# abb128/april-asr

Hardware: AMD Instinct MI355X
Metric: audio_seconds_per_second (concurrent 16 kHz sessions x 1/RTF), aprilv0_en-us-sized streaming RNN-T (higher is better)
Workload: dtype f32

## Files before the change

### april_asr_amd/csrc/engine.cc

```cpp
#include "engine.h"
#include <array>
#include <algorithm>
#include <cmath>
#include <chrono>
#include <cstdlib>
#include <cstring>
#include "common.h"
#include "env.h"

namespace aprilx {

static size_t align64(size_t x) { return (x + 63) & ~(size_t)63; }

void plan_layout(const NetDims &d, bool has_dec_conv_b, PackedLayout &L)
{
    L.dims = d;
    L.has_dec_conv_b = has_dec_conv_b;
    L.vocab_pad = (d.vocab + 31) & ~31;
    size_t off = 0;
    auto take = [&](size_t n) { size_t o = off; off = align64(off + n); return o; };
    L.k3 = (d.conv_ch[1] * 9 + 63) & ~63;
    L.conv_w[0] = take((size_t)d.conv_ch[0] * 9); L.conv_b[0] = take((size_t)d.conv_ch[0]);
    L.conv_w[1] = take((size_t)d.conv_ch[1] * d.conv_ch[0] * 9); L.conv_b[1] = take((size_t)d.conv_ch[1]);
    L.conv_w[2] = take((size_t)L.k3 * d.conv_ch[2]); L.conv_b[2] = take((size_t)d.conv_ch[2]);
    L.w_embed = take((size_t)d.embed_in * d.d_model); L.b_embed = take((size_t)d.d_model);
    L.layers.resize((size_t)d.n_layers);
    for (auto &l : L.layers) {
        l.wg = take((size_t)2 * d.d_model * 4 * d.hidden); l.bg = take((size_t)4 * d.hidden);
        l.whr = take((size_t)d.hidden * d.d_model);
        l.wff1 = take((size_t)d.d_model * d.ffn); l.bff1 = take((size_t)d.ffn);
        l.wff2 = take((size_t)d.ffn * d.d_model); l.bff2 = take((size_t)d.d_model);
    }
    L.w_encproj = take((size_t)d.d_model * d.joiner); L.b_encproj = take((size_t)d.joiner);
    L.emb = take((size_t)d.vocab * d.d_model);
    L.dec_conv = take((size_t)d.d_model * (d.d_model / d.dec_groups) * d.context);
    L.dec_conv_b = take((size_t)d.d_model);
    L.w_decproj = take((size_t)d.d_model * d.joiner); L.b_decproj = take((size_t)d.joiner);
    L.w_out = take((size_t)d.joiner * L.vocab_pad); L.b_out = take((size_t)L.vocab_pad);
    L.total = off;
}

std::vector<std::pair<size_t, size_t>> gemm_sections(const PackedLayout &L)
{
    const NetDims &d = L.dims;
    std::vector<std::pair<size_t, size_t>> v;
    v.emplace_back(L.w_embed, (size_t)d.embed_in * d.d_model);
    for (const PackedLayout::Layer &o : L.layers) {
        v.emplace_back(o.wg, (size_t)2 * d.d_model * 4 * d.hidden); v.emplace_back(o.whr, (size_t)d.hidden * d.d_model);
        v.emplace_back(o.wff1, (size_t)d.d_model * d.ffn); v.emplace_back(o.wff2, (size_t)d.ffn * d.d_model);
    }
    v.emplace_back(L.w_encproj, (size_t)d.d_model * d.joiner); v.emplace_back(L.w_decproj, (size_t)d.d_model * d.joiner);
    v.emplace_back(L.w_out, (size_t)d.joiner * L.vocab_pad);
    return v;
}

static void pack_mfma(const float *W, int K, int N, int Npad, const std::vector<int> *colmap, float *dst)
{
    const int KB = K / 16, NTt = Npad / 16;
    for (int t = 0; t < NTt; ++t)
        for (int kb = 0; kb < KB; ++kb)
            for (int lane = 0; lane < 64; ++lane) {
                const int np = t * 16 + (lane & 15);
                const int src = np < N ? (colmap ? (*colmap)[(size_t)np] : np) : -1;
                float *o = dst + (((size_t)t * KB + kb) * 64 + lane) * 4;
                for (int j = 0; j < 4; ++j) {
                    const int k = kb * 16 + (lane >> 4) * 4 + j;
                    o[j] = src >= 0 ? W[(size_t)k * N + src] : 0.0f;
                }
            }
}

void pack_weights(const HostModel &m, PackedLayout &L, std::vector<float> &blob)
{
    const NetDims &d = L.dims;
    blob.assign(L.total, 0.0f);
    float *B = blob.data();
    for (int i = 0; i < 3; ++i) {
        if (i < 2) memcpy(B + L.conv_w[i], m.conv_w[i].data(), m.conv_w[i].size() * 4);
        memcpy(B + L.conv_b[i], m.conv_b[i].data(), m.conv_b[i].size() * 4);
    }
    {
        const int kreal = d.conv_ch[1] * 9, c2 = d.conv_ch[2];
        std::vector<float> w3((size_t)L.k3 * c2, 0.0f);
        for (int o = 0; o < c2; ++o) for (int k = 0; k < kreal; ++k) w3[(size_t)k * c2 + o] = m.conv_w[2][(size_t)o * kreal + k];
        pack_mfma(w3.data(), L.k3, c2, c2, nullptr, B + L.conv_w[2]);
    }
    {
        const int c2 = d.conv_ch[2], F = d.f_out;
        std::vector<float> we((size_t)d.embed_in * d.d_model);
        for (int c = 0; c < c2; ++c) for (int f = 0; f < F; ++f)
            memcpy(&we[((size_t)f * c2 + c) * d.d_model], &m.w_embed[((size_t)c * F + f) * d.d_model], (size_t)d.d_model * 4);
        pack_mfma(we.data(), d.embed_in, d.d_model, d.d_model, nullptr, B + L.w_embed);
    }
    memcpy(B + L.b_embed, m.b_embed.data(), (size_t)d.d_model * 4);
    L.embed_eps = m.embed_norm_eps;
    L.norm_eps.resize((size_t)d.n_layers);
    std::vector<int> gmap((size_t)4 * d.hidden);
    for (int u = 0; u < d.hidden; ++u) for (int g = 0; g < 4; ++g) gmap[(size_t)u * 4 + g] = g * d.hidden + u;
    for (int l = 0; l < d.n_layers; ++l) {
        const LayerWeights &lw = m.layers[(size_t)l];
        const PackedLayout::Layer &o = L.layers[(size_t)l];
        pack_mfma(lw.w_gates.data(), 2 * d.d_model, 4 * d.hidden, 4 * d.hidden, &gmap, B + o.wg);
        for (int n = 0; n < 4 * d.hidden; ++n) B[o.bg + n] = lw.b_gates[(size_t)gmap[(size_t)n]];
        pack_mfma(lw.w_hr.data(), d.hidden, d.d_model, d.d_model, nullptr, B + o.whr);
        pack_mfma(lw.w_ff1.data(), d.d_model, d.ffn, d.ffn, nullptr, B + o.wff1);
        memcpy(B + o.bff1, lw.b_ff1.data(), (size_t)d.ffn * 4);
        pack_mfma(lw.w_ff2.data(), d.ffn, d.d_model, d.d_model, nullptr, B + o.wff2);
        memcpy(B + o.bff2, lw.b_ff2.data(), (size_t)d.d_model * 4);
        L.norm_eps[(size_t)l] = lw.norm_eps;
    }
    pack_mfma(m.w_encproj.data(), d.d_model, d.joiner, d.joiner, nullptr, B + L.w_encproj);
    memcpy(B + L.b_encproj, m.b_encproj.data(), (size_t)d.joiner * 4);
    memcpy(B + L.emb, m.emb.data(), m.emb.size() * 4);
    memcpy(B + L.dec_conv, m.dec_conv.data(), m.dec_conv.size() * 4);
    if (!m.dec_conv_b.empty()) memcpy(B + L.dec_conv_b, m.dec_conv_b.data(), m.dec_conv_b.size() * 4);
    pack_mfma(m.w_decproj.data(), d.d_model, d.joiner, d.joiner, nullptr, B + L.w_decproj);
    memcpy(B + L.b_decproj, m.b_decproj.data(), (size_t)d.joiner * 4);
    pack_mfma(m.w_out.data(), d.joiner, d.vocab, L.vocab_pad, nullptr, B + L.w_out);
    memcpy(B + L.b_out, m.b_out.data(), (size_t)d.vocab * 4);
}

template <typename T> static T *dmalloc(size_t n) { HipLegacyLock legacy; T *p = nullptr; HIP_CHECK(hipMalloc((void **)&p, std::max<size_t>(n, 1) * sizeof(T))); return p; }
template <typename T> static T *hmalloc(size_t n) { HipLegacyLock legacy; T *p = nullptr; HIP_CHECK(hipHostMalloc((void **)&p, std::max<size_t>(n, 1) * sizeof(T), hipHostMallocDefault)); return p; }

std::recursive_mutex &hip_legacy_mutex() { static std::recursive_mutex m; return m; }

static int pick_kz(int K, int N, int kblk = 16)
{
    int kz = 256 / std::max(1, N / 16);
    kz = std::max(1, std::min(kz, 8));
    while (kz > 1 && ((K / kblk) / kz < 4 || (K / kblk) % (4 * kz) != 0)) kz >>= 1;
    return kz;
}

Engine::Engine(const EngineConfig &cfg, const PackedLayout &layout, const float *blob_host, const float *blob_device,
               const ModelParams &params, const FbankHostTables &ft, const std::vector<uint8_t> &tok_class)
    : cfg_(cfg), L_(layout), P_(params)
{
    HipLegacyLock legacy;
    HIP_CHECK(hipSetDevice(cfg_.device));
    HIP_CHECK(hipStreamCreateWithFlags(&stream_, hipStreamNonBlocking));
    HIP_CHECK(hipStreamCreateWithFlags(&f_stream_, hipStreamNonBlocking));
    HIP_CHECK(hipStreamCreateWithFlags(&s_stream_, hipStreamNonBlocking));
    search_stream_ = stream_;
    for (int i = 0; i < 32; ++i) { hipEvent_t e; HIP_CHECK(hipEventCreateWithFlags(&e, hipEventDisableTiming)); join_ev_.push_back(e); }
    split_streams_ = std::max(0, std::min(2, env_int("APRIL_SPLIT_STREAMS", 2)));
    const NetDims &d = L_.dims;
    w_ = dmalloc<float>(L_.total);
    if (blob_device) HIP_CHECK(hipMemcpy(w_, blob_device, L_.total * 4, hipMemcpyDeviceToDevice));
    else if (blob_host) HIP_CHECK(hipMemcpy(w_, blob_host, L_.total * 4, hipMemcpyHostToDevice));

    const size_t S = (size_t)cfg_.max_slots, MB = (size_t)cfg_.max_batch;
    ring_frames_ = std::max(P_.segment_size * 32, env_int("APRIL_RING_FRAMES", 8192));
    h_ = dmalloc<float>((size_t)d.n_layers * S * d.d_model);
    c_ = dmalloc<float>((size_t)d.n_layers * S * d.hidden);
    if (!env_str("APRIL_RING_FRAMES")) {
        size_t free_b = 0, total_b = 0;
        if (hipMemGetInfo(&free_b, &total_b) == hipSuccess && free_b > 0) {
            const size_t per_frame = S * (size_t)d.mel * sizeof(float);
            const size_t fit = (free_b / 4) / per_frame;
            if (fit < (size_t)ring_frames_) {
                const int shrunk = std::max(P_.segment_size * 32, (int)std::min<size_t>(fit, 8192) / 64 * 64);
                LOGW("engine: %zu MB of feature rings (%d frames x %zu slots) exceed a quarter of the %zu MB free on device %d: %d frames per session",
                     per_frame * (size_t)ring_frames_ >> 20, ring_frames_, S, free_b >> 20, cfg_.device, shrunk);
                ring_frames_ = shrunk;
            }
        } else (void)hipGetLastError();
        float *p = nullptr;
        if (hipMalloc((void **)&p, S * ring_frames_ * d.mel * sizeof(float)) == hipSuccess) ring_ = p;
        else {
            (void)hipGetLastError();
            const size_t asked = S * (size_t)ring_frames_ * d.mel * sizeof(float);
            ring_frames_ = std::max(P_.segment_size * 32, 2048);
            LOGW("engine: no room for %zu MB of feature rings, falling back to %d frames per session", asked >> 20, ring_frames_);
        }
    }
    if (!ring_) ring_ = dmalloc<float>(S * ring_frames_ * d.mel);
    eout_ = dmalloc<float>(S * d.joiner);
    dout_ = dmalloc<float>(S * d.joiner);
    gstate_ = dmalloc<GreedyState>(S);
    HIP_CHECK(hipMemset(h_, 0, (size_t)d.n_layers * S * d.d_model * 4));
    HIP_CHECK(hipMemset(c_, 0, (size_t)d.n_layers * S * d.hidden * 4));
    HIP_CHECK(hipMemset(ring_, 0, S * ring_frames_ * d.mel * 4));
    HIP_CHECK(hipMemset(eout_, 0, S * d.joiner * 4));
    HIP_CHECK(hipMemset(dout_, 0, S * d.joiner * 4));
    {
        std::vector<GreedyState> init(S);
        for (auto &g : init) { g.ctx0 = P_.blank_id; g.ctx1 = P_.blank_id; g.last_tok = -1; g.last_emit_ms = 0; }
        HIP_CHECK(hipMemcpy(gstate_, init.data(), S * sizeof(GreedyState), hipMemcpyHostToDevice));
    }
    cls_ = dmalloc<uint8_t>((size_t)d.vocab);
    HIP_CHECK(hipMemcpy(cls_, tok_class.data(), (size_t)d.vocab, hipMemcpyHostToDevice));

    kz_embed_ = pick_kz(d.embed_in, d.d_model);
    kz_hr_ = pick_kz(d.hidden, d.d_model);
    kz_ff2_ = pick_kz(d.ffn, d.d_model);
    kz_proj_ = pick_kz(d.d_model, d.joiner);
    kz_out_ = pick_kz(d.joiner, L_.vocab_pad);
    {
        const bool want = cfg_.precision == 1 && env_int("APRIL_F16_TILE", 1) != 0;
        f16_tile_ = want && d.d_model % 128 == 0 && d.hidden % 128 == 0 && d.ffn % 128 == 0 && d.hidden % 16 == 0;
        if (f16_tile_) {
            kzx_hr_ = pick_kz(d.hidden, d.d_model, 32); kzx_ff2_ = pick_kz(d.ffn, d.d_model, 32);
            for (int p = 0; p < 2; ++p) y16_buf_[p] = dmalloc<uint16_t>(MB * d.d_model);
            y16_ = y16_buf_[0];
            for (int p = 0; p < 2; ++p) { xb16_buf_[p] = dmalloc<uint16_t>(MB * d.d_model); u16_buf_[p] = dmalloc<uint16_t>(MB * d.hidden); ff16_buf_[p] = dmalloc<uint16_t>(MB * d.ffn); }
            xb16_ = xb16_buf_[0]; u16_ = u16_buf_[0]; ff16_ = ff16_buf_[0];
            h16_ = dmalloc<uint16_t>((size_t)d.n_layers * S * d.d_model);
            HIP_CHECK(hipMemset(h16_, 0, (size_t)d.n_layers * S * d.d_model * 2));
        }
    }
    ws_mstride_ = cfg_.max_batch;
    const size_t ws_n = (size_t)std::max({kz_embed_ * d.d_model, kz_hr_ * d.d_model, kz_ff2_ * d.d_model, kz_proj_ * d.joiner, kz_out_ * L_.vocab_pad});
    ws_ = dmalloc<float>(ws_n * MB);
    ws_g_ = dmalloc<float>((size_t)std::max(kz_proj_ * d.joiner, kz_out_ * L_.vocab_pad) * MB);
    xin_ = dmalloc<float>(MB * d.embed_in);
    a3_ = dmalloc<float>(MB * d.f_out * L_.k3);
    HIP_CHECK(hipMemset(a3_, 0, MB * d.f_out * L_.k3 * 4));
    for (int p = 0; p < 2; ++p) { y_buf_[p] = dmalloc<float>(MB * d.d_model); ssq_buf_[p] = dmalloc<float>(MB * (d.d_model / SSQ_COLS)); }
    y_ = y_buf_[0]; ssq_ = ssq_buf_[0];
    ws_fe_ = dmalloc<float>((size_t)kz_embed_ * d.d_model * MB);
    ws_sr_ = dmalloc<float>((size_t)std::max(kz_proj_ * d.joiner, d.d_model) * MB);
    for (int p = 0; p < 2; ++p) { xb_buf_[p] = dmalloc<float>(MB * d.d_model); u_buf_[p] = dmalloc<float>(MB * d.hidden); ff_buf_[p] = dmalloc<float>(MB * d.ffn); }
    xb_ = xb_buf_[0]; u_ = u_buf_[0]; ff_ = ff_buf_[0];
    ramp_mode_ = env_int("APRIL_RAMP_MERGE", 1);
    if (ramp_mode_ < 0 || ramp_mode_ > 2) ramp_mode_ = 1;
    ramp_d_ = dmalloc<RampState>(1); HIP_CHECK(hipMemset(ramp_d_, 0, sizeof(RampState)));
    de_ = dmalloc<float>(MB * d.d_model);
    HIP_CHECK(hipMemset(de_, 0, MB * d.d_model * 4));
    logits_ = dmalloc<float>(3 * MB * d.vocab);
    logits_h_ = hmalloc<float>(3 * MB * d.vocab);
    ring_cap_ = std::max<size_t>((size_t)1 << 20, 3 * MB * 8 + 2 * S); ring_h_ = hmalloc<int>(2 * ring_cap_);
    step_cap_ = 1 << 14; step_off_h_ = hmalloc<int>((size_t)2 * step_cap_); rec_off_h_ = hmalloc<int>((size_t)2 * step_cap_);
    rec_cap_ = std::max<size_t>((size_t)1 << 20, 3 * MB * 8); rec_d_ = dmalloc<StepRecord>(2 * rec_cap_); rec_h_ = hmalloc<StepRecord>(2 * rec_cap_);
    for (int i = 0; i < 2; ++i) HIP_CHECK(hipEventCreateWithFlags(&flight_done_[i], hipEventDisableTiming));
    counter_d_ = dmalloc<int>(1);
    for (int p = 0; p < 2; ++p) {
        rec_off_buf_[p] = dmalloc<int>(1); flags_buf_[p] = dmalloc<int>(8); step_buf_[p] = dmalloc<int>(4 * MB);
        HIP_CHECK(hipMemset(rec_off_buf_[p], 0, 4)); HIP_CHECK(hipMemset(flags_buf_[p], 0, 32));
    }
    rec_off_d_ = rec_off_buf_[0]; flags_d_ = flags_buf_[0]; step_d_ = step_buf_[0];
    active_d_ = dmalloc<int>(MB); dirty_d_ = dmalloc<int>(MB);
    dec_slots_d_ = dmalloc<int>(std::max(S, MB));
    HIP_CHECK(hipMemset(counter_d_, 0, 4));

    upload_tables(ft);
    use_graphs_ = env_int("APRIL_NO_GRAPHS", 0) == 0;
    if (const int n = env_int("APRIL_GRAPH_CACHE_CAP", 0))
        step_graphs_.cap = lm_graphs_.cap = lm_search_graphs_.cap = sw_plan_cap_ = (size_t)std::max(n, 2), sw_graphs_.cap = 4 * sw_plan_cap_;
    free_.reserve(S);
    for (int i = cfg_.max_slots - 1; i >= 0; --i) free_.push_back(i);
    LOGI("engine: device %d, %d slots, max batch %d, weights %.1f MB, kz(embed,hr,ff2,proj,out)=%d,%d,%d,%d,%d",
         cfg_.device, cfg_.max_slots, cfg_.max_batch, L_.total * 4.0 / 1e6, kz_embed_, kz_hr_, kz_ff2_, kz_proj_, kz_out_);
}

void Engine::finish_weights()
{
    HipLegacyLock legacy;
    HIP_CHECK(hipSetDevice(cfg_.device));
    if (cfg_.precision == 1 && !wh_) {
        wh_ = dmalloc<uint16_t>(L_.total);
        for (const auto &sec : gemm_sections(L_)) launch_cvt_f16(w_ + sec.first, wh_ + sec.first, sec.second, nullptr);
        if (f16_tile_) {
            const NetDims &d = L_.dims;
            wx_ = dmalloc<uint16_t>(L_.total);
            for (const PackedLayout::Layer &o : L_.layers) {
                launch_repack_x32(w_ + o.wg, wx_ + o.wg, 2 * d.d_model, 4 * d.hidden, nullptr);
                launch_repack_x32(w_ + o.whr, wx_ + o.whr, d.hidden, d.d_model, nullptr);
                launch_repack_x32(w_ + o.wff1, wx_ + o.wff1, d.d_model, d.ffn, nullptr);
                launch_repack_x32(w_ + o.wff2, wx_ + o.wff2, d.ffn, d.d_model, nullptr);
            }
        }
        HIP_CHECK(hipDeviceSynchronize());
    }
    if (!conv_wt_) {
        const NetDims &d = L_.dims;
        conv_wt_ = dmalloc<float>((size_t)9 * d.conv_ch[0] + (size_t)9 * d.conv_ch[0] * d.conv_ch[1]);
        launch_conv_weight_transpose(w_ + L_.conv_w[0], w_ + L_.conv_w[1], d.conv_ch[0], d.conv_ch[1], conv_wt_, conv_wt_ + (size_t)9 * d.conv_ch[0], nullptr);
        HIP_CHECK(hipDeviceSynchronize());
    }
    build_dec_table();
}

void Engine::build_dec_table()
{
    if (dec_table_) return;
    const NetDims &d = L_.dims;
    const size_t limit_mb = (size_t)std::max(0, env_int("APRIL_DEC_TABLE_MB", 2048));
    const size_t rows = (size_t)d.vocab * (size_t)d.vocab;
    if (d.context != 2 || rows * (size_t)d.joiner * 4 > limit_mb * 1024 * 1024 || rows * (size_t)d.joiner * 4 >= ((size_t)1 << 32)) return;
    const int MB = cfg_.max_batch;
    float *table = dmalloc<float>(rows * (size_t)d.joiner);
    std::vector<int> iota((size_t)MB), ctx((size_t)MB * 2);
    for (int i = 0; i < MB; ++i) iota[(size_t)i] = i;
    int *ctx_d = dmalloc<int>((size_t)MB * 2);
    HIP_CHECK(hipMemcpy(dec_slots_d_, iota.data(), (size_t)MB * 4, hipMemcpyHostToDevice));
    for (size_t base = 0; base < rows; base += (size_t)MB) {
        const int n = (int)std::min<size_t>((size_t)MB, rows - base);
        for (int i = 0; i < n; ++i) { const size_t r = base + (size_t)i; ctx[(size_t)2 * i] = (int)(r / (size_t)d.vocab); ctx[(size_t)2 * i + 1] = (int)(r % (size_t)d.vocab); }
        HIP_CHECK(hipMemcpy(ctx_d, ctx.data(), (size_t)n * 8, hipMemcpyHostToDevice));
        DecEmbedArgs a; a.dec = dec_params(); a.ctx = ctx_d; a.M = n; a.out = de_; a.ldo = d.d_model;
        launch_dec_embed(a, stream_);
        run_decproj(n, dec_slots_d_, nullptr, nullptr, 1, table + base * (size_t)d.joiner);
        HIP_CHECK(hipStreamSynchronize(stream_));
    }
    (void)hipFree(ctx_d);
    dec_table_ = table;
    LOGI("engine: decoder table %zu rows x %d (%.0f MB)", rows, d.joiner, rows * (double)d.joiner * 4 / 1e6);
}

Engine::~Engine()
{
    HipLegacyLock legacy;
    (void)hipSetDevice(cfg_.device);
    (void)hipStreamSynchronize(f_stream_); (void)hipStreamSynchronize(stream_); (void)hipStreamSynchronize(s_stream_);
    dump_stream_trace();
    if (ramp_d_ && ramp_eligible_.load() > 0) {
        unsigned h = 0;
        if (hipMemcpy(&h, &ramp_d_->hosted, sizeof h, hipMemcpyDeviceToHost) == hipSuccess) LOGI("engine: ramp merge: %u of %llu hostable split feeds were hosted by their predecessor", h, (unsigned long long)ramp_eligible_.load());
    }
    for (StreamTrace &t : trace_) for (hipEvent_t e : t.ev) if (e) (void)hipEventDestroy(e);
    if (trace_base_) (void)hipEventDestroy(trace_base_);
    for (hipEvent_t e : join_ev_) (void)hipEventDestroy(e);
    for (auto &e : ev_pool_) { (void)hipEventDestroy(e.a); (void)hipEventDestroy(e.b); }
    drop_graphs(); free_sw_plans(); if (gclk_slots_) (void)hipFree(gclk_slots_);
    if (lm_stream_) { (void)hipStreamSynchronize(lm_stream_); (void)hipStreamDestroy(lm_stream_); }
    for (hipEvent_t e : lm_events_) (void)hipEventDestroy(e);
    if (zargs_h_) { (void)hipHostFree(zargs_h_); (void)hipFree(zargs_d_); }
    for (int i = 0; i < 3; ++i) if (zargs_done_[i]) (void)hipEventDestroy(zargs_done_[i]);
    for (void *p : {(void *)lm_now_d_, (void *)lm_rows_d_, (void *)lm_rec_off_d_}) if (p) (void)hipFree(p);
    if (conf_k_d_) (void)hipFree(conf_k_d_);
    if (conf_d_) (void)hipFree(conf_d_);
    if (conf_k_h_) (void)hipHostFree(conf_k_h_);
    if (conf_h_) (void)hipHostFree(conf_h_);
    for (auto &b : bias_sets_) if (b.dev) (void)hipFree(b.dev);
    for (void *p : {(void *)bias_set_d_, (void *)bias_state_d_, (void *)bias_desc_d_}) if (p) (void)hipFree(p);
    for (void *p : {(void *)bias_set_h_, (void *)bias_desc_h_}) if (p) (void)hipHostFree(p);
    if (opt_d_) (void)hipFree(opt_d_);
    if (opt_h_) (void)hipHostFree(opt_h_);
    if (ws_g_) (void)hipFree(ws_g_);
    if (conv_wt_) (void)hipFree(conv_wt_);
    if (dec_table_) (void)hipFree(dec_table_);
    if (p_lm_) (void)hipFree(p_lm_);
    for (int p = 0; p < 2; ++p)
        for (void *q : {(void *)eout_lm_buf_[p], (void *)y16_buf_[p], (void *)y_buf_[p], (void *)ssq_buf_[p], (void *)xb_buf_[p], (void *)u_buf_[p], (void *)ff_buf_[p],
                        (void *)xb16_buf_[p], (void *)u16_buf_[p], (void *)ff16_buf_[p], (void *)rec_off_buf_[p], (void *)flags_buf_[p], (void *)step_buf_[p]}) if (q) (void)hipFree(q);
    if (ws_fe_) (void)hipFree(ws_fe_);
    if (ws_sr_) (void)hipFree(ws_sr_);
    for (void *p : {(void *)wx_, (void *)h16_, (void *)ramp_d_}) if (p) (void)hipFree(p);
    for (void *p : {(void *)w_, (void *)wh_, (void *)h_, (void *)c_, (void *)ring_, (void *)eout_, (void *)dout_, (void *)gstate_, (void *)cls_, (void *)ws_, (void *)xin_,
                    (void *)a3_, (void *)de_, (void *)logits_, (void *)rec_d_, (void *)counter_d_,
                    (void *)active_d_, (void *)dirty_d_, (void *)dec_slots_d_,
                    (void *)ds_desc_[0], (void *)ds_desc_[1], (void *)ds_pcm_[0], (void *)ds_pcm_[1]})
        if (p) (void)hipFree(p);
    for (void *p : {(void *)ring_h_, (void *)step_off_h_, (void *)rec_off_h_, (void *)rec_h_, (void *)logits_h_, (void *)hs_desc_[0], (void *)hs_desc_[1], (void *)hs_pcm_[0], (void *)hs_pcm_[1]})
        if (p) (void)hipHostFree(p);
    for (int b = 0; b < 2; ++b) if (fb_done_[b]) (void)hipEventDestroy(fb_done_[b]);
    for (int b = 0; b < 2; ++b) if (flight_done_[b]) (void)hipEventDestroy(flight_done_[b]);
    for (void *p : table_allocs_) (void)hipFree(p);
    (void)hipStreamDestroy(stream_); (void)hipStreamDestroy(f_stream_); (void)hipStreamDestroy(s_stream_);
}

void Engine::upload_tables(const FbankHostTables &ft)
{
    auto up = [&](const void *src, size_t bytes) {
        void *p = nullptr;
        HIP_CHECK(hipMalloc(&p, std::max<size_t>(bytes, 16)));
        if (bytes) HIP_CHECK(hipMemcpy(p, src, bytes, hipMemcpyHostToDevice));
        table_allocs_.push_back(p);
        return p;
    };
    ft_.window = (const float *)up(ft.window.data(), ft.window.size() * 4);
    ft_.mel = (const float *)up(ft.mel.data(), ft.mel.size() * 4);
    ft_.mel_lo = (const int *)up(ft.mel_lo.data(), ft.mel_lo.size() * 4);
    ft_.mel_hi = (const int *)up(ft.mel_hi.data(), ft.mel_hi.size() * 4);
    ft_.nfct = (int)ft.factors.size();
    for (int k = 0; k < ft_.nfct; ++k) {
        ft_.fct[k] = ft.factors[(size_t)k];
        ft_.tw[k] = (const double *)up(ft.tw[(size_t)k].data(), ft.tw[(size_t)k].size() * 8);
        ft_.tws[k] = ft.tws[(size_t)k].empty() ? nullptr : (const double *)up(ft.tws[(size_t)k].data(), ft.tws[(size_t)k].size() * 8);
    }
    ft_.padded = ft.padded; ft_.nbins = ft.nbins;
    pad_value_ = ft.pad_value;
}

int Engine::alloc_slot()
{
    std::lock_guard<std::mutex> g(slot_mu_);
    if (free_.empty() && !zero_pending_.empty()) zero_pending_slots();
    if (free_.empty()) return -1;
    const int s = free_.back();
    free_.pop_back();
    ++live_;
    return s;
}

void Engine::zero_pending_slots()
{
    if (zero_pending_.empty()) return;
    if (hipSetDevice(cfg_.device) == hipSuccess) {
        std::lock_guard<std::mutex> cg(capture_mu_);
        m_touched();
        const NetDims &d = L_.dims;
        for (size_t o = 0; o < zero_pending_.size(); o += 64) {
            ZeroSlotArgs z;
            z.h = h_; z.c = c_; z.n_layers = d.n_layers; z.slots = (size_t)cfg_.max_slots; z.d_model = d.d_model; z.hidden = d.hidden;
            z.eout = eout_; z.dout = dout_; z.joiner = d.joiner; z.state = gstate_; z.blank = P_.blank_id; z.h16 = h16_;
            z.n_list = (int)std::min<size_t>(64, zero_pending_.size() - o);
            for (int i = 0; i < z.n_list; ++i) z.list[i] = zero_pending_[o + (size_t)i];
            launch_zero_slot(z, stream_);
        }
    }
    for (int s : zero_pending_) free_.push_back(s);
    zero_pending_.clear();
}

void Engine::free_slot(int slot)
{
    if (conf_ever_.load(std::memory_order_relaxed)) set_slot_confidence(slot, 0);
    if (bias_ever_.load(std::memory_order_relaxed)) set_slot_bias(slot, nullptr);
    if (opt_ever_.load(std::memory_order_relaxed)) set_slot_search_options(slot, SearchOpt{0u, 0.0f});
    std::lock_guard<std::mutex> g(slot_mu_);
    zero_pending_.push_back(slot);
    --live_;
    if (zero_pending_.size() >= 256) zero_pending_slots();
}

void Engine::sync_streams()
{
    HIP_CHECK(hipStreamSynchronize(f_stream_)); HIP_CHECK(hipStreamSynchronize(stream_)); HIP_CHECK(hipStreamSynchronize(s_stream_));
}

void Engine::sync()
{
    m_touched();
    sync_streams();
    f_unseen_by_m_ = s_unseen_by_m_ = m_unseen_by_f_ = m_unseen_by_s_ = false;
    if (profiling_) collect_timing();
}

template <typename Chain> static hipGraphExec_t capture_graph(hipStream_t st, Chain &&chain)
{
    hipGraph_t graph = nullptr;
    hipGraphExec_t exec = nullptr;
    HipLegacyLock capture_guard;
    HIP_CHECK(hipStreamBeginCapture(st, hipStreamCaptureModeRelaxed));
    chain();
    HIP_CHECK(hipStreamEndCapture(st, &graph));
    HIP_CHECK(hipGraphInstantiate(&exec, graph, nullptr, nullptr, 0));
    HIP_CHECK(hipGraphDestroy(graph));
    return exec;
}

void GraphCache::clear()
{
    if (!map_.empty()) LOGI("engine: %s graphs emptied (%zu entries)", name, map_.size());
    for (auto &g : map_) (void)hipGraphExecDestroy(g.second);
    map_.clear(); uses_.clear();
}

template <typename Chain> hipGraphExec_t Engine::cached_graph(GraphCache &cache, const GraphCache::Key &key, hipStream_t st, Chain &&chain)
{
    if (!cache.find(key)) cache.insert(key, capture_graph(st, chain));
    return cache.find(key);
}

template <typename Capture> void Engine::capture_both_parities(Capture &&capture)
{
    const int par = flight_parity_;
    m_touched();
    for (int q : {1 - par, par}) { select_parity(q); capture(); }
}

Engine::StreamTrace *Engine::trace_slot()
{
    static const char *path = env_str("APRIL_STREAM_TRACE");
    if (!path) return nullptr;
    if (!trace_base_) { HIP_CHECK(hipEventCreate(&trace_base_)); HIP_CHECK(hipEventRecord(trace_base_, stream_)); }
    if (trace_.size() >= 4096) return nullptr;
    trace_.emplace_back();
    StreamTrace &t = trace_.back();
    for (hipEvent_t &e : t.ev) HIP_CHECK(hipEventCreate(&e));
    return &t;
}

void Engine::dump_stream_trace()
{
    const char *path = env_str("APRIL_STREAM_TRACE");
    if (!path || trace_.empty()) return;
    FILE *f = fopen(path, "w");
    if (!f) return;
    fprintf(f, "# one line per split feed; times in us since the first split feed; FE = index fetch + conv + embed on stream F, LY = layer wavefront on M, SR = encoder_proj + search on S\n");
    fprintf(f, "# feed sessions chunks  FE_start FE_end  LY_start LY_end  SR_start SR_end   overlap: FE inside the previous feed's LY window? SR inside the next feed's LY window?\n");
    std::vector<std::array<float, 6>> ts;
    for (StreamTrace &t : trace_) {
        std::array<float, 6> a{};
        bool ok = t.used;
        for (int i = 0; i < 6 && ok; ++i) ok = hipEventElapsedTime(&a[(size_t)i], trace_base_, t.ev[i]) == hipSuccess;
        if (ok) ts.push_back(a); else (void)hipGetLastError();
    }
    for (size_t i = 0; i < ts.size(); ++i) {
        const auto &a = ts[i];
        const bool fe_in_prev = i > 0 && a[0] * 1e3f < ts[i - 1][3] * 1e3f && a[1] * 1e3f > ts[i - 1][2] * 1e3f;
        const bool sr_in_next = i + 1 < ts.size() && a[5] > ts[i + 1][2] && a[4] < ts[i + 1][3];
        fprintf(f, "%4zu %5d %2d  %10.1f %10.1f  %10.1f %10.1f  %10.1f %10.1f   %s %s\n", i, trace_[i].m, trace_[i].T, a[0] * 1e3, a[1] * 1e3, a[2] * 1e3, a[3] * 1e3, a[4] * 1e3, a[5] * 1e3,
                fe_in_prev ? "FE<prevLY" : "-", sr_in_next ? "SR<nextLY" : "-");
    }
    fclose(f);
}

void Engine::join(hipStream_t waiter, hipStream_t src)
{
    hipEvent_t e = join_ev_[join_pos_++ % join_ev_.size()];
    HIP_CHECK(hipEventRecord(e, src));
    HIP_CHECK(hipStreamWaitEvent(waiter, e, 0));
}

void Engine::general_prologue()
{
    m_touched();
    if (f_unseen_by_m_) { join(stream_, f_stream_); f_unseen_by_m_ = false; }
    if (s_unseen_by_m_) { join(stream_, s_stream_); s_unseen_by_m_ = false; }
    m_unseen_by_f_ = m_unseen_by_s_ = true;
    flight_tail_s_ = false;
}

void Engine::set_profiling(bool on) { std::lock_guard<std::mutex> cg(capture_mu_); sync(); profiling_ = on; }
void Engine::reset_timing() { for (auto &t : timing_) t = KernelTiming(); }
void Engine::set_gates_clock(bool on)
{
    std::lock_guard<std::mutex> cg(capture_mu_);
    HIP_CHECK(hipSetDevice(cfg_.device));
    sync();
    if (on) {
        if (!gclk_slots_) gclk_slots_ = dmalloc<unsigned long long>((size_t)GCLK_SLOTS * STAMP_WORDS);
        HIP_CHECK(hipMemsetAsync(gclk_slots_, 0, (size_t)GCLK_SLOTS * STAMP_WORDS * 8, stream_));
        HIP_CHECK(hipStreamSynchronize(stream_));
        gclk_ms_ = 0; gclk_launches_ = 0; gclk_rows_ = 0;
        for (int i = 0; i < 4; ++i) { gclk_ms_n_[i] = 0; gclk_launches_n_[i] = 0; }
        gclk_ = true;
        return;
    }
    collect_gates_clock(); gclk_ = false;
}
void Engine::collect_gates_clock()
{
    if (!gclk_ || !gclk_slots_) return;
    std::vector<unsigned long long> h((size_t)GCLK_SLOTS * STAMP_WORDS);
    HIP_CHECK(hipMemcpyAsync(h.data(), gclk_slots_, h.size() * 8, hipMemcpyDeviceToHost, stream_)); HIP_CHECK(hipStreamSynchronize(stream_));
    for (auto &kv : sw_plans_)
        for (size_t i = 0; i < kv.second.stamp_slots.size(); ++i) {
            const auto &sl = kv.second.stamp_slots[i];
            const unsigned long long ticks = h[(size_t)sl.first * STAMP_WORDS + 2], n = h[(size_t)sl.first * STAMP_WORDS + 3];
            gclk_ms_ += (double)ticks * 1e-5; gclk_launches_ += (long)n; gclk_rows_ += (long)n * sl.second;
            const int bn = std::min(std::max(kv.second.stamp_n[i], 1), 4) - 1;
            gclk_ms_n_[bn] += (double)ticks * 1e-5; gclk_launches_n_[bn] += (long)n;
        }
}
void Engine::timed_begin(int cls)
{
    ++launch_count_;
    if (!profiling_) return;
    if (ev_used_ == ev_pool_.size()) { Ev e; HIP_CHECK(hipEventCreate(&e.a)); HIP_CHECK(hipEventCreate(&e.b)); e.cls = cls; ev_pool_.push_back(e); }
    ev_pool_[ev_used_].cls = cls;
    if (cls == T_GATES) gemm_profile_next_launch(ev_pool_[ev_used_].a, ev_pool_[ev_used_].b);
    else HIP_CHECK(hipEventRecord(ev_pool_[ev_used_].a, stream_));
}
void Engine::timed_end(int cls)
{
    if (!profiling_) return;
    if (cls == T_GATES) {
        if (gemm_profile_pending()) { gemm_profile_next_launch(nullptr, nullptr); return; }
    } else HIP_CHECK(hipEventRecord(ev_pool_[ev_used_].b, stream_));
    ++ev_used_;
}
void Engine::collect_timing()
{
    for (size_t i = 0; i < ev_used_; ++i) {
        float ms = 0;
        if (hipEventElapsedTime(&ms, ev_pool_[i].a, ev_pool_[i].b) == hipSuccess) { timing_[ev_pool_[i].cls].ms += ms; timing_[ev_pool_[i].cls].launches++; }
    }
    ev_used_ = 0;
}

void Engine::fbank(int n_frames, const FbankFrameDesc *desc, const std::pair<const int16_t *, size_t> *parts, size_t n_parts, size_t n_pcm, HostPool *pool)
{
    const int n_rs = n_frames > 0 ? std::max(rs_n_, 0) : 0;
    ResampleDesc *rs = rs_desc_;
    const std::pair<const int16_t *, size_t> *in_parts = rs_in_parts_;
    const size_t n_in_parts = n_rs ? rs_n_in_parts_ : 0, n_in = n_rs ? rs_n_in_ : 0;
    rs_n_ = 0;
    const int n_dc = n_frames > 0 ? std::max(dc_n_, 0) : 0;
    const DecodeDesc *dc = dc_desc_;
    const std::pair<const uint8_t *, size_t> *raw_parts = dc_raw_parts_;
    const size_t n_raw_parts = n_dc ? dc_n_raw_parts_ : 0, n_raw = n_dc ? dc_n_raw_ : 0;
    const size_t raw_units = n_dc ? (n_raw + 1) / 2 + 8 : 0;
    dc_n_ = 0;
    if (n_frames <= 0) return;
    HIP_CHECK(hipSetDevice(cfg_.device));
    for (int i = 0; i < n_rs; ++i) rs[i].taps = resample_table(rs_specs_[i]);
    if (n_frames > desc_cap_ || n_pcm + n_in + raw_units > pcm_cap_ || (size_t)n_rs > rs_cap_ || (size_t)n_dc > dc_cap_) {
        sync();
        HipLegacyLock regrow_guard;
        for (int b = 0; b < 2; ++b) {
            if (hs_desc_[b]) { (void)hipHostFree(hs_desc_[b]); (void)hipFree(ds_desc_[b]); }
            if (hs_pcm_[b]) { (void)hipHostFree(hs_pcm_[b]); (void)hipFree(ds_pcm_[b]); }
        }
        desc_cap_ = std::max({n_frames * 2, desc_cap_, 1024});
        pcm_cap_ = std::max({(n_pcm + n_in + raw_units) * 2, pcm_cap_, (size_t)1 << 16});
        rs_cap_ = std::max({(size_t)n_rs * 2, rs_cap_, n_rs ? (size_t)256 : (size_t)0});
        dc_cap_ = std::max({(size_t)n_dc * 2, dc_cap_, n_dc ? (size_t)256 : (size_t)0});
        const size_t units = pcm_cap_ + 8 + ((size_t)desc_cap_ * sizeof(FbankFrameDesc) + 1) / 2 + 8 + rs_cap_ * sizeof(ResampleDesc) / 2
                             + 8 + dc_cap_ * sizeof(DecodeDesc) / 2;
        for (int b = 0; b < 2; ++b) {
            hs_pcm_[b] = hmalloc<int16_t>(units); ds_pcm_[b] = dmalloc<int16_t>(units);
            hs_desc_[b] = nullptr; ds_desc_[b] = nullptr;
            if (!fb_done_[b]) HIP_CHECK(hipEventCreateWithFlags(&fb_done_[b], hipEventDisableTiming));
        }
    }
    const int b = fb_flip_;
    fb_flip_ ^= 1;
    HIP_CHECK(hipEventSynchronize(fb_done_[b]));
    const size_t woff = ((n_pcm + n_in) * sizeof(int16_t) + 15) / 16 * 16;
    const size_t doff = (woff + n_raw + 15) / 16 * 16;
    const size_t roff = (doff + (size_t)n_frames * sizeof(FbankFrameDesc) + 15) / 16 * 16;
    const size_t coff = (roff + (size_t)n_rs * sizeof(ResampleDesc) + 15) / 16 * 16;
    const size_t bytes = n_dc ? coff + (size_t)n_dc * sizeof(DecodeDesc)
                              : (n_rs ? roff + (size_t)n_rs * sizeof(ResampleDesc) : doff + (size_t)n_frames * sizeof(FbankFrameDesc));
    char *hs = reinterpret_cast<char *>(hs_pcm_[b]);
    memcpy(hs + doff, desc, (size_t)n_frames * sizeof(FbankFrameDesc));
    ResampleArgs ra;
    if (n_rs) {
        ResampleDesc *hr = reinterpret_cast<ResampleDesc *>(hs + roff);
        int64_t blocks = 0, lds = 0;
        for (int i = 0; i < n_rs; ++i) {
            hr[i] = rs[i];
            hr[i].in_off += (int32_t)n_pcm;
            blocks = std::max<int64_t>(blocks, (rs[i].out_cnt + kResampleBlock - 1) / kResampleBlock);
            lds = std::max<int64_t>(lds, resample_lds_floats(rs[i].L, rs[i].M, rs[i].K));
        }
        ra.n_desc = n_rs; ra.max_blocks = (int)blocks; ra.lds_floats = (int)lds;
    }
    DecodeArgs da;
    if (n_dc) {
        DecodeDesc *hd = reinterpret_cast<DecodeDesc *>(hs + coff);
        int64_t blocks = 0; uint64_t frames = 0;
        for (int i = 0; i < n_dc; ++i) {
            hd[i] = dc[i];
            if (dc[i].dst_in) hd[i].dst += (int32_t)n_pcm;
            blocks = std::max<int64_t>(blocks, (dc[i].out_cnt + kDecodeBlock - 1) / kDecodeBlock);
            frames += (uint64_t)dc[i].n_src;
        }
        da.n_desc = n_dc; da.max_blocks = (int)blocks;
        dc_launches_.fetch_add(1, std::memory_order_relaxed); dc_frames_.fetch_add(frames, std::memory_order_relaxed);
    }
    auto stage = [&](const auto *pp, size_t np, size_t base) {
        const size_t el = sizeof(*pp[0].first);
        char *dst = hs;
        if (pool && np >= 256) {
            part_off_.resize(np);
            size_t off = base;
            for (size_t i = 0; i < np; ++i) { part_off_[i] = off; off += pp[i].second; }
            pool->run(np, 64, [&](size_t i) { if (pp[i].first) memcpy(dst + part_off_[i] * el, pp[i].first, pp[i].second * el); });
        } else {
            size_t off = base;
            for (size_t i = 0; i < np; ++i) { if (pp[i].first) memcpy(dst + off * el, pp[i].first, pp[i].second * el); off += pp[i].second; }
        }
    };
    stage(parts, n_parts, 0);
    if (n_in_parts) stage(in_parts, n_in_parts, n_pcm);
    if (n_raw_parts) stage(raw_parts, n_raw_parts, woff);
    std::lock_guard<std::mutex> cg(capture_mu_);
    if (m_unseen_by_f_) { join(f_stream_, stream_); m_unseen_by_f_ = false; }
    HIP_CHECK(hipMemcpyAsync(ds_pcm_[b], hs_pcm_[b], bytes, hipMemcpyHostToDevice, f_stream_));
    FbankArgs a;
    a.t = ft_; a.pcm = ds_pcm_[b]; a.desc = reinterpret_cast<const FbankFrameDesc *>(reinterpret_cast<const char *>(ds_pcm_[b]) + doff); a.n_frames = n_frames; a.ring = ring_; a.ring_frames = ring_frames_; a.pad_value = pad_value_;
    if (n_rs) { ra.in = ds_pcm_[b]; ra.out = ds_pcm_[b]; ra.desc = reinterpret_cast<const ResampleDesc *>(reinterpret_cast<const char *>(ds_pcm_[b]) + roff); }
    if (n_dc) {
        da.raw = reinterpret_cast<const uint8_t *>(ds_pcm_[b]) + woff; da.out = ds_pcm_[b];
        da.desc = reinterpret_cast<const DecodeDesc *>(reinterpret_cast<const char *>(ds_pcm_[b]) + coff);
    }
    if (profiling_) {
        m_touched();
        join(stream_, f_stream_);
        if (n_dc) { timed_begin(T_DECODE); launch_decode(da, stream_); timed_end(T_DECODE); }
        if (n_rs) { timed_begin(T_RESAMPLE); launch_resample(ra, stream_); timed_end(T_RESAMPLE); }
        timed_begin(T_FBANK); launch_fbank(a, stream_); timed_end(T_FBANK);
        join(f_stream_, stream_);
    } else {
        if (n_dc) launch_decode(da, f_stream_);
        if (n_rs) launch_resample(ra, f_stream_);
        launch_fbank(a, f_stream_);
    }
    HIP_CHECK(hipEventRecord(fb_done_[b], f_stream_));
    f_unseen_by_m_ = true;
}

const float *Engine::resample_table(const ResampleSpec *spec)
{
    std::lock_guard<std::mutex> g(rs_mu_);
    auto it = rs_tables_.find(spec);
    if (it != rs_tables_.end()) return it->second;
    HIP_CHECK(hipSetDevice(cfg_.device));
    float *d = dmalloc<float>(spec->taps.size());
    {
        HipLegacyLock legacy;
        if (!spec->taps.empty()) HIP_CHECK(hipMemcpy(d, spec->taps.data(), spec->taps.size() * sizeof(float), hipMemcpyHostToDevice));
        table_allocs_.push_back(d);
    }
    rs_tables_[spec] = d;
    return d;
}


RowScale Engine::in_scale(int l, size_t r0) const
{
    const NetDims &d = L_.dims;
    const int G = d.d_model / SSQ_COLS;
    RowScale r; r.ssq = ssq_ + r0 * G; r.groups = G; r.inv_n = 1.0f / (float)(d.d_norm ? d.d_norm : d.d_model); r.eps = l == 0 ? L_.embed_eps : L_.norm_eps[(size_t)l - 1];
    return r;
}

GemmArgs Engine::args_gates(int l, size_t r0, int rows, int waves) const
{
    const NetDims &d = L_.dims;
    const size_t S = (size_t)cfg_.max_slots;
    const PackedLayout::Layer &o = L_.layers[(size_t)l];
    GemmArgs g; g.a0 = y_ + r0 * d.d_model; g.lda0 = d.d_model; g.K0 = d.d_model; g.lda1 = d.d_model; g.K1 = d.d_model;
    lin(g, o.wg); g.M = rows; g.N = 4 * d.hidden; g.K = 2 * d.d_model; g.kz = 1; g.wave_mask = waves;
    if (f16_tile_) { g.a0 = reinterpret_cast<const float *>(y16_ + r0 * d.d_model); lin16(g, o.wg); }
    if (waves != GATES_H) g.x_scale = in_scale(l, r0);
    if (waves == GATES_X) {
        g.a1 = g.a0; g.epi = EPI_XPART; g.out = p_lm_ + r0 * 4 * d.hidden; g.ldo = 4 * d.hidden;
        return g;
    }
    g.a1 = h_ + (size_t)l * S * d.d_model; g.aidx1 = step_d_; g.epi = EPI_LSTM;
    g.out = u_ + r0 * d.hidden; g.ldo = d.hidden; g.bias = w_ + o.bg; g.c_state = c_ + (size_t)l * S * d.hidden; g.slot_idx = step_d_; g.hidden = d.hidden;
    if (waves == GATES_H) { g.p_add = p_lm_ + r0 * 4 * d.hidden; g.ldp = 4 * d.hidden; }
    else if (cfg_.precision == 0 && gates_tile_rows(rows)) g.tile_ok = 2;
    if (f16_tile_) {
        g.a1 = reinterpret_cast<const float *>(h16_ + (size_t)l * S * d.d_model); g.out = nullptr; g.out16 = u16_ + r0 * d.hidden;
    }
    return g;
}

constexpr long GATES_TILE_MIN_ROWS = 2048;
bool Engine::gates_tile_rows(long rows) const
{
    static const int mode = env_int("APRIL_GATES_TILE", 2);
    return mode == 1 || (mode == 2 && rows >= GATES_TILE_MIN_ROWS);
}

GemmArgs Engine::args_whr(int l, size_t r0, int rows) const
{
    const NetDims &d = L_.dims;
    const size_t S = (size_t)cfg_.max_slots;
    const PackedLayout::Layer &o = L_.layers[(size_t)l];
    GemmArgs g; g.a0 = u_ + r0 * d.hidden; g.lda0 = d.hidden; g.K0 = d.hidden; lin(g, o.whr);
    g.M = rows; g.N = d.d_model; g.K = d.hidden; g.kz = kz_hr_; g.tile_ok = tile_ok(); g.force_fullk = 1;
    g.epi = EPI_HR; g.state = h_ + (size_t)l * S * d.d_model; g.ld_state = d.d_model; g.slot_idx = step_d_; g.resid = y_ + r0 * d.d_model; g.ldr = d.d_model;
    g.r_scale = in_scale(l, r0);
    g.out = xb_ + r0 * d.d_model; g.ldo = d.d_model;
    if (f16_tile_) {
        g.a0 = reinterpret_cast<const float *>(u16_ + r0 * d.hidden); lin16(g, o.whr); g.kz = kzx_hr_;
        g.state16 = h16_ + (size_t)l * S * d.d_model; g.out16 = xb16_ + r0 * d.d_model;
    }
    return g;
}

GemmArgs Engine::args_ff1(int l, size_t r0, int rows) const
{
    const NetDims &d = L_.dims;
    const PackedLayout::Layer &o = L_.layers[(size_t)l];
    GemmArgs g; g.a0 = xb_ + r0 * d.d_model; g.lda0 = d.d_model; g.K0 = d.d_model; lin(g, o.wff1);
    g.M = rows; g.N = d.ffn; g.K = d.d_model; g.kz = 1; g.epi = EPI_BIAS_DSWISH; g.out = ff_ + r0 * d.ffn; g.ldo = d.ffn; g.bias = w_ + o.bff1;
    if (f16_tile_) { g.a0 = reinterpret_cast<const float *>(xb16_ + r0 * d.d_model); lin16(g, o.wff1); g.out = nullptr; g.out16 = ff16_ + r0 * d.ffn; }
    return g;
}

GemmArgs Engine::args_ff2(int l, size_t r0, int rows) const
{
    const NetDims &d = L_.dims;
    const PackedLayout::Layer &o = L_.layers[(size_t)l];
    GemmArgs g; g.a0 = ff_ + r0 * d.ffn; g.lda0 = d.ffn; g.K0 = d.ffn; lin(g, o.wff2);
    g.M = rows; g.N = d.d_model; g.K = d.ffn; g.kz = kz_ff2_; g.tile_ok = tile_ok(); g.force_fullk = 1;
    g.epi = EPI_RESID_SSQ; g.bias = w_ + o.bff2; g.resid = xb_ + r0 * d.d_model; g.ldr = d.d_model; g.out = y_ + r0 * d.d_model; g.ldo = d.d_model; g.ssq_out = ssq_ + r0 * (d.d_model / SSQ_COLS);
    if (f16_tile_) { g.a0 = reinterpret_cast<const float *>(ff16_ + r0 * d.ffn); lin16(g, o.wff2); g.kz = kzx_ff2_; g.out16 = y16_ + r0 * d.d_model; }
    return g;
}

GemmArgs Engine::args_encproj(size_t r0, int rows, const int *slot_idx, float *out) const
{
    const NetDims &d = L_.dims;
    GemmArgs g; g.a0 = y_ + r0 * d.d_model; g.lda0 = d.d_model; g.K0 = d.d_model; lin(g, L_.w_encproj);
    g.M = rows; g.N = d.joiner; g.K = d.d_model; g.kz = kz_proj_; g.tile_ok = tile_ok();
    g.epi = EPI_SLOT_STORE; g.bias = w_ + L_.b_encproj; g.out = out; g.ldo = d.joiner; g.slot_idx = slot_idx; g.x_scale = in_scale(d.n_layers, r0);
    return g;
}

static GemmArgs partial_form(const GemmArgs &f, float *ws, int m_stride)
{
    GemmArgs g = f;
    g.epi = EPI_PARTIAL; g.force_fullk = 0; g.out = ws; g.m_stride = m_stride;
    g.bias = nullptr; g.resid = nullptr; g.state = nullptr; g.slot_idx = nullptr; g.ssq_out = nullptr; g.r_scale = RowScale(); g.out16 = nullptr; g.state16 = nullptr;
    g.x_scale = RowScale(); g.row_mask = nullptr;
    return g;
}
static RowArgs row_form(const GemmArgs &f, const float *ws, int m_stride, int parts)
{
    RowArgs r; r.ws = ws; r.parts = parts; r.m_stride = m_stride; r.N = f.N; r.M = f.M;
    r.resid = f.resid; r.ldr = f.ldr; r.out = f.out; r.ldo = f.ldo; r.out16 = f.out16; r.run_flag = f.run_flag; r.run_gen = f.run_gen;
    if (f.epi == EPI_HR) { r.mode = ROW_HR; r.r_scale = f.r_scale; r.slot_idx = f.slot_idx; r.state = f.state; r.ld_state = f.ld_state; r.state16 = f.state16; }
    else if (f.epi == EPI_RESID_SSQ) { r.mode = ROW_RESID_SSQ; r.bias = f.bias; r.ssq_out = f.ssq_out; }
    else { r.mode = ROW_SLOT_STORE; r.bias = f.bias; r.slot_idx = f.slot_idx; r.r_scale = f.x_scale; r.row_mask = f.row_mask; }
    return r;
}

void Engine::launch_rowepi(GemmArgs f, float *ws, hipStream_t st, bool force, int cls)
{
    const int row_cls = cls == T_DEC ? T_DEC : T_ROW;
    f.force_fullk = force ? 1 : 0;
    if (gemm_fullk(f.M, f.N, f.kz, force, 1, f.tile_ok)) { timed_begin(cls); launch_gemm(f, st); timed_end(cls); return; }
    timed_begin(cls); launch_gemm(partial_form(f, ws, ws_mstride_), st); timed_end(cls);
    timed_begin(row_cls); launch_row(row_form(f, ws, ws_mstride_, gemm_partials(f.M, f.N, f.kz, 1, f.tile_ok)), st); timed_end(row_cls);
}

void Engine::encoder_front(size_t r0, int rows, const int *row_slots, const float *x_direct, hipStream_t st, float *ws)
{
    const NetDims &d = L_.dims;
    ConvEmbedArgs ca;
    ca.ring = ring_; ca.ring_frames = ring_frames_; ca.mel = d.mel; ca.seg = d.seg;
    ca.slot_idx = row_slots + r0; ca.ring_tail = step_d_ + cfg_.max_batch + r0; ca.x_direct = x_direct;
    for (int i = 0; i < 3; ++i) { ca.w[i] = w_ + L_.conv_w[i]; ca.b[i] = w_ + L_.conv_b[i]; ca.ch[i] = d.conv_ch[i]; ca.stride[i] = d.conv_stride[i]; }
    ca.ch1_per_group = 1;
    for (int k = 8; k > 1; --k) if (d.conv_ch[1] % k == 0) { ca.ch1_per_group = k; break; }
    ca.out = a3_ + r0 * d.f_out * L_.k3; ca.ldo = L_.k3; ca.M = rows;
    if (conv_wt_) { ca.w0t = conv_wt_; ca.w1t = conv_wt_ + (size_t)9 * d.conv_ch[0]; }
    timed_begin(T_CONV); launch_conv_embed(ca, st); timed_end(T_CONV);
    {
        GemmArgs g; g.a0 = ca.out; g.lda0 = L_.k3; g.K0 = L_.k3; g.wp = w_ + L_.conv_w[2];
        g.M = rows * d.f_out; g.N = d.conv_ch[2]; g.K = L_.k3; g.kz = 1; g.epi = EPI_BIAS_DSWISH; g.out = xin_ + r0 * d.embed_in; g.ldo = d.conv_ch[2]; g.bias = w_ + L_.conv_b[2];
        timed_begin(T_CONV); launch_gemm(g, st); timed_end(T_CONV);
    }
    {
        GemmArgs g; g.a0 = xin_ + r0 * d.embed_in; g.lda0 = d.embed_in; g.K0 = d.embed_in; lin(g, L_.w_embed);
        g.M = rows; g.N = d.d_model; g.K = d.embed_in; g.kz = kz_embed_; g.tile_ok = tile_ok();
        g.epi = EPI_RESID_SSQ; g.bias = w_ + L_.b_embed; g.ldr = d.d_model; g.out = y_ + r0 * d.d_model; g.ldo = d.d_model; g.ssq_out = ssq_ + r0 * (d.d_model / SSQ_COLS);
        launch_rowepi(g, ws + r0 * d.d_model, st);
    }
    if (f16_tile_) launch_cvt_f16(y_ + r0 * d.d_model, y16_ + r0 * d.d_model, (size_t)rows * d.d_model, st);
}

void Engine::run_encoder_rows(int n, const float *x_direct)
{
    const NetDims &d = L_.dims;
    encoder_front(0, n, step_d_, x_direct, stream_, ws_);
    for (int l = 0; l < d.n_layers; ++l) {
        timed_begin(T_GATES); launch_gemm(args_gates(l, 0, n, GATES_ALL), stream_); timed_end(T_GATES);
        launch_rowepi(args_whr(l, 0, n), ws_, stream_);
        timed_begin(T_GEMM_OTHER); launch_gemm(args_ff1(l, 0, n), stream_); timed_end(T_GEMM_OTHER);
        launch_rowepi(args_ff2(l, 0, n), ws_, stream_);
    }
    launch_rowepi(args_encproj(0, n, step_d_, eout_), ws_, stream_);
}

DecEmbedParams Engine::dec_params() const
{
    const NetDims &d = L_.dims;
    DecEmbedParams p; p.emb = w_ + L_.emb; p.conv_w = w_ + L_.dec_conv; p.conv_b = L_.has_dec_conv_b ? w_ + L_.dec_conv_b : nullptr;
    p.d = d.d_model; p.groups = d.dec_groups; p.context = d.context; p.vocab = d.vocab;
    return p;
}

void Engine::run_decproj(int n, const int *d_slots, const int *row_mask, const int *run_flag, int run_gen, float *out)
{
    const NetDims &d = L_.dims;
    GemmArgs g; g.a0 = de_; g.lda0 = d.d_model; g.K0 = d.d_model; lin(g, L_.w_decproj);
    g.M = n; g.N = d.joiner; g.K = d.d_model; g.kz = kz_proj_; g.tile_ok = tile_ok(); g.run_flag = run_flag; g.run_gen = run_gen;
    g.epi = EPI_SLOT_STORE; g.bias = w_ + L_.b_decproj; g.out = out ? out : dout_; g.ldo = d.joiner; g.slot_idx = d_slots; g.row_mask = row_mask;
    launch_rowepi(g, ws_g_, search_stream_, false, T_DEC);
}

void Engine::run_greedy_rounds(int n, bool dump_logits, int chunk, const float *eout_rows)
{
    const int MB = cfg_.max_batch;
    GreedyIo io;
    io.gen = chunk + 1; io.now = step_d_ + 2 * MB + (size_t)chunk * n; io.eout = eout_rows; io.rec_off = rec_off_d_; io.rec_slot0 = chunk * 3;
    io.dump = dump_logits ? logits_ + (size_t)chunk * 3 * n * L_.dims.vocab : nullptr;
    run_greedy_rounds(n, io);
}

void Engine::run_greedy_rounds(int n, const GreedyIo &io)
{
    const NetDims &d = L_.dims;
    const int gen = io.gen;
    const int *d_slots = step_d_;
    for (int round = 0; round < 3; ++round) {
        {
            GemmArgs g; g.a0b = dout_; g.lda0 = d.joiner; g.K0 = d.joiner; g.a_op = AOP_TANH_ADD;
            if (dec_table_) { g.a0b = dec_table_; g.ctx_state = gstate_; g.ctx_vocab = d.vocab; }
            if (io.eout) { g.a0 = io.eout; g.aidx0 = io.eout_rows; g.same_idx_b = 0; g.aidx0b = d_slots; }
            else { g.a0 = eout_; g.aidx0 = d_slots; }
            lin(g, L_.w_out); g.M = n; g.N = L_.vocab_pad; g.K = d.joiner; g.kz = kz_out_; g.epi = EPI_PARTIAL; g.out = ws_g_; g.m_stride = ws_mstride_;
            if (round > 0) { g.run_flag = flags_d_ + round; g.run_gen = gen; }
            timed_begin(T_DEC); launch_gemm(g, search_stream_); timed_end(T_DEC);
        }
        DecideArgs a;
        a.ws = ws_g_; a.parts = gemm_partials(n, L_.vocab_pad, kz_out_); a.m_stride = ws_mstride_; a.N = L_.vocab_pad; a.M = n; a.n_valid = d.vocab;
        a.bias = w_ + L_.b_out; a.blank = P_.blank_id; a.early_emit = round == 0 ? 1.0f : 0.0f;
        a.slot_idx = d_slots; a.now_ms = io.now; a.active = active_d_; a.dirty = dirty_d_; a.tok_class = cls_; a.state = gstate_;
        a.rec_ring = rec_d_; a.rec_off = io.rec_off; a.round = round; a.gen = gen; a.rec_slot = io.rec_slot0 + round;
        a.logits_dump = io.dump ? io.dump + (size_t)round * n * d.vocab : nullptr;
        a.dec = dec_params(); a.de_out = dec_table_ ? nullptr : de_; a.ld_de = d.d_model;
        a.run_flags = flags_d_; a.rerun_flags = flags_d_ + 4;
        a.conf_k = conf_k_d_; a.conf_ring = conf_d_;
        a.bias_set = bias_set_d_; a.bias_state = bias_state_d_; a.bias_desc = bias_desc_d_;
        a.opt = opt_d_;
        timed_begin(T_DEC); launch_decide(a, search_stream_); timed_end(T_DEC);
        if (!dec_table_) run_decproj(n, d_slots, dirty_d_, flags_d_ + 4 + round, gen);
    }
}

AdvanceArgs Engine::advance_args(int m, int T) const
{
    AdvanceArgs a;
    a.host_ring = ring_h_; a.host_step_off = step_off_h_; a.host_rec_off = rec_off_h_; a.counter = counter_d_; a.index_mask = 2 * step_cap_ - 1;
    a.dst = step_d_; a.dst_stride = cfg_.max_batch; a.n_arrays = T ? 4 : 3; a.len[0] = m;
    for (int i = 1; i < a.n_arrays; ++i) a.len[i] = T ? m * T : m;
    a.rec_off = rec_off_d_; a.flags = flags_d_; a.n_flags = 8;
    return a;
}

void Engine::run_chain(int m, bool dump_logits)
{
    launch_advance(advance_args(m, 0), stream_);
    run_encoder_rows(m, nullptr);
    run_greedy_rounds(m, dump_logits);
}

void Engine::lm_stage_layer(int l, int m, int t0, int t1, hipStream_t st)
{
    const NetDims &d = L_.dims;
    const size_t b0 = (size_t)t0 * m;
    const int brows = (t1 - t0) * m;
    timed_begin(T_GATES); launch_gemm(args_gates(l, b0, brows, GATES_X), st); timed_end(T_GATES);
    for (int t = t0; t < t1; ++t) {
        const size_t r0 = (size_t)t * m;
        timed_begin(T_GATES); launch_gemm(args_gates(l, r0, m, GATES_H), st); timed_end(T_GATES);
        launch_rowepi(args_whr(l, r0, m), ws_ + r0 * d.d_model, st, !f16_tile_);
    }
    timed_begin(T_GEMM_OTHER); launch_gemm(args_ff1(l, b0, brows), st); timed_end(T_GEMM_OTHER);
    launch_rowepi(args_ff2(l, b0, brows), ws_ + b0 * d.d_model, st);
}

void Engine::lm_stage_proj(int m, int t0, int t1, hipStream_t st, float *ws)
{
    const NetDims &d = L_.dims;
    const size_t b0 = (size_t)t0 * m;
    launch_rowepi(args_encproj(b0, (t1 - t0) * m, nullptr, eout_lm_ + b0 * d.joiner), ws + b0 * d.d_model, st, true);
}

static int lm_block_steps(int T)
{
    const int b = (int)(0.75 * std::sqrt((double)std::max(1, T)) + 0.5);
    return std::max(6, std::min(32, b));
}
constexpr int LM_WAVEFRONT_MIN_CHUNKS = 10;

static bool lm_wavefront_on()
{
    static const bool on = env_int("APRIL_LM_WAVEFRONT", 1) != 0;
    return on;
}

void Engine::run_lm_chain(int m, int T, bool dump_logits)
{
    const NetDims &d = L_.dims;
    const int MB = cfg_.max_batch;
    const int L = d.n_layers;
    launch_advance(advance_args(m, T), stream_);
    encoder_front(0, m * T, step_d_ + 3 * MB, nullptr, stream_, ws_);
    for (int l = 0; l < L; ++l) lm_stage_layer(l, m, 0, T, stream_);
    lm_stage_proj(m, 0, T, stream_, ws_);
    for (int t = 0; t < T; ++t) run_greedy_rounds(m, dump_logits, t, eout_lm_ + (size_t)t * m * d.joiner);
}

void Engine::run_lm_wavefront(int m, int T, bool dump_logits)
{
    const NetDims &d = L_.dims;
    const int MB = cfg_.max_batch;
    const int L = d.n_layers;
    const int blk = lm_block_steps(T);
    const int NB = (T + blk - 1) / blk;
    launch_advance(advance_args(m, T), stream_);
    hipStream_t cs = lm_stream_;
    HIP_CHECK(hipEventRecord(lm_events_[0], stream_));
    HIP_CHECK(hipStreamWaitEvent(cs, lm_events_[0], 0));

    const size_t need = (size_t)(NB + L + 1) * (size_t)(2 * blk + 6) * (size_t)L;
    if (need > zargs_region_) {
        HIP_CHECK(hipStreamSynchronize(cs));
        HipLegacyLock regrow_guard;
        if (zargs_h_) { (void)hipHostFree(zargs_h_); (void)hipFree(zargs_d_); }
        zargs_region_ = need + need / 4;
        zargs_h_ = hmalloc<GemmArgs>(3 * zargs_region_); zargs_d_ = dmalloc<GemmArgs>(3 * zargs_region_);
        for (int i = 0; i < 3; ++i) zargs_busy_[i] = false;
    }
    const int zslot = zargs_next_;
    zargs_next_ = (zargs_next_ + 1) % 3;
    if (zargs_busy_[zslot]) HIP_CHECK(hipEventSynchronize(zargs_done_[zslot]));
    zargs_pos_ = (size_t)zslot * zargs_region_;

    static const bool timing = env_str("APRIL_LM_TIMING") != nullptr;
    double tacc[6] = {0, 0, 0, 0, 0, 0};
    auto now = [&]() { return timing ? std::chrono::duration<double, std::micro>(std::chrono::steady_clock::now().time_since_epoch()).count() : 0.0; };
    struct Batch { size_t off; int n; };
    std::vector<Batch> plan;
    std::vector<size_t> plan_end((size_t)(NB + L + 1), 0);
    std::vector<GemmArgs> items;
    struct Act { int l, t0, t1; };
    std::vector<Act> act;
    double tq = now();
    auto lap = [&](int i) { if (timing) { const double t = now(); tacc[i] += t - tq; tq = t; } };
    const size_t first = zargs_pos_;
    for (int W = 0; W <= NB + L; ++W) {
        act.clear();
        for (int l = 0; l < L; ++l) { const int b = W - 1 - l; if (b >= 0 && b < NB) act.push_back({l, b * blk, std::min(T, (b + 1) * blk)}); }
        auto flush = [&]() {
            if (items.empty()) return;
            stage_gemm_z(items.data(), (int)items.size(), zargs_h_ + zargs_pos_);
            plan.push_back({zargs_pos_, (int)items.size()});
            zargs_pos_ += items.size(); items.clear();
        };
        auto by_len = [&](auto make) {
            for (int pass = 0; pass < 2; ++pass) {
                for (const Act &x : act) if (((x.t1 - x.t0) == blk) == (pass == 0)) items.push_back(make(x));
                flush();
            }
        };
        by_len([&](const Act &x) { return args_gates(x.l, (size_t)x.t0 * m, (x.t1 - x.t0) * m, GATES_X); });
        for (int i = 0; i < blk; ++i) {
            for (const Act &x : act) if (x.t0 + i < x.t1) items.push_back(args_gates(x.l, (size_t)(x.t0 + i) * m, m, GATES_H));
            flush();
            for (const Act &x : act) if (x.t0 + i < x.t1) items.push_back(args_whr(x.l, (size_t)(x.t0 + i) * m, m));
            flush();
        }
        by_len([&](const Act &x) { return args_ff1(x.l, (size_t)x.t0 * m, (x.t1 - x.t0) * m); });
        by_len([&](const Act &x) { return args_ff2(x.l, (size_t)x.t0 * m, (x.t1 - x.t0) * m); });
        plan_end[(size_t)W] = plan.size();
    }
    lap(0);
    if (zargs_pos_ > first)
        HIP_CHECK(hipMemcpyAsync(zargs_d_ + first, zargs_h_ + first, (zargs_pos_ - first) * sizeof(GemmArgs), hipMemcpyHostToDevice, cs));
    lap(1);
    for (int W = 0; W <= NB + L; ++W) {
        if (W < NB) encoder_front((size_t)W * blk * m, (std::min(T, (W + 1) * blk) - W * blk) * m, step_d_ + 3 * MB, nullptr, cs, ws_);
        lap(2);
        for (size_t k = W ? plan_end[(size_t)W - 1] : 0; k < plan_end[(size_t)W]; ++k) launch_gemm_z(zargs_h_ + plan[k].off, plan[k].n, zargs_d_ + plan[k].off, cs);
        lap(3);
        const int bp = W - L - 1;
        if (bp >= 0) {
            const int t0 = bp * blk, t1 = std::min(T, t0 + blk), len = t1 - t0;
            lm_stage_proj(m, t0, t1, cs, ws_);
            hipEvent_t e = lm_events_[1 + (size_t)(bp % (int)(lm_events_.size() - 1))];
            HIP_CHECK(hipEventRecord(e, cs));
            HIP_CHECK(hipStreamWaitEvent(stream_, e, 0));
            BlockSetupArgs bs;
            bs.now_src = step_d_ + 2 * MB + (size_t)t0 * m; bs.now_dst = lm_now_d_; bs.rows_dst = lm_rows_d_; bs.row0 = t0 * m; bs.count = len * m;
            bs.rec_off_step = rec_off_d_; bs.rec_off_block = lm_rec_off_d_; bs.rec_add = t0 * 3 * m; bs.flags = flags_d_; bs.n_flags = 8;
            launch_block_setup(bs, stream_);
            lap(4);
            auto search = [&]() {
                for (int i = 0; i < len; ++i) {
                    GreedyIo io;
                    io.gen = i + 1; io.now = lm_now_d_ + (size_t)i * m; io.eout = eout_lm_; io.eout_rows = lm_rows_d_ + (size_t)i * m;
                    io.rec_off = lm_rec_off_d_; io.rec_slot0 = i * 3;
                    io.dump = dump_logits ? logits_ + (size_t)(t0 + i) * 3 * m * d.vocab : nullptr;
                    run_greedy_rounds(m, io);
                }
            };
            if (!use_graphs_ || dump_logits) { search(); continue; }
            const GraphCache::Key key = graph_key(m, len);
            if (!lm_search_graphs_.find(key) && lm_search_graphs_.full()) { HIP_CHECK(hipStreamSynchronize(stream_));  lm_search_graphs_.clear(); }
            HIP_CHECK(hipGraphLaunch(cached_graph(lm_search_graphs_, key, stream_, search), stream_));
            lap(5);
        }
    }
    HIP_CHECK(hipEventRecord(zargs_done_[zslot], cs));
    zargs_busy_[zslot] = true;
    if (timing) fprintf(stderr, "lm wavefront %d x %d: host us: args %.0f, arg copy %.0f, front end %.0f, layer launches %.0f, proj + events + setup %.0f, search graph %.0f\n",
                        m, T, tacc[0], tacc[1], tacc[2], tacc[3], tacc[4], tacc[5]);
}

static bool lm_gates_split_on()
{
    static const bool on = env_int("APRIL_GATES_SPLIT", 1) != 0;
    return on;
}

Engine::SwPlan &Engine::sw_plan(int m, int T)
{
    const GraphCache::Key key = sw_key(m, T);
    auto it = sw_plans_.find(key);
    if (it != sw_plans_.end()) return it->second;
    if (sw_plans_.size() >= sw_plan_cap_) {
        sync();
        HipLegacyLock evict_guard;
        collect_gates_clock(); free_sw_plans();
        if (gclk_slots_) { HIP_CHECK(hipMemsetAsync(gclk_slots_, 0, (size_t)GCLK_SLOTS * STAMP_WORDS * 8, stream_)); HIP_CHECK(hipStreamSynchronize(stream_)); }
        gclk_used_ = 0;
    }
    SwPlan &p = sw_plans_[key];
    build_sw_chain(p, p.one, m, T, false);
    if (ramp_mode_ != 0 && !gclk_) build_sw_chain(p, p.split, m, T, true);
    return p;
}

std::vector<RampStep> ramp_window(int L, int T, int R, int max_problems)
{
    std::vector<RampStep> w;
    if (L <= 2 * R || T < 1 || R < 1) return w;
    for (int j = 1; j <= R; ++j) {
        RampStep s; s.macro = L + T - 1 - R + j;
        for (int l = 0; l < L; ++l) { const int t = s.macro - 1 - l; if (t >= 0 && t < T) ++s.own; }
        for (int t = 0; t < j; ++t) s.guests.push_back(std::make_pair(j - 1 - t, t));
        if (s.own + (int)s.guests.size() > max_problems) return std::vector<RampStep>();
        w.push_back(s);
    }
    return w;
}

void Engine::ramp_counts(uint64_t *hosted, uint64_t *eligible)
{
    unsigned h = 0;
    {
        HipLegacyLock legacy;
        if (hipSetDevice(cfg_.device) == hipSuccess) HIP_CHECK(hipMemcpy(&h, &ramp_d_->hosted, sizeof h, hipMemcpyDeviceToHost));
    }
    *hosted = h; *eligible = ramp_eligible_.load(std::memory_order_relaxed);
}

void Engine::build_sw_chain(SwPlan &p, SwPlan::Chain &c, int m, int T, bool ramp)
{
    const NetDims &d = L_.dims;
    const int L = d.n_layers;
    const int par = flight_parity_;
    const int tk = f16_tile_ ? 2 : tile_ok();
    auto needs_rows = [&](int kind, int n) {
        const int kz = kind == 1 ? kz_hr() : kz_ff2();
        return (kind == 1 || kind == 3) && tk && (tk == 2 || gemm_tile_planned(m, d.d_model, kz, n)) && !gemm_fullk(m, d.d_model, kz, false, n, tk);
    };
    std::vector<RampStep> window;
    if (ramp && m <= RAMP_MAX_M && T <= RAMP_MAX_T) {
        window = ramp_window(L, T, RAMP_R);
        for (const RampStep &s : window) if (needs_rows(1, s.own + (int)s.guests.size()) || needs_rows(3, s.own + (int)s.guests.size())) { window.clear(); break; }
    }
    if (ramp) p.hosts = !window.empty();
    std::vector<GemmArgs> items;
    std::vector<RowArgs> rows;
    for (int W = 0; W <= T + L; ++W) {
        const RampStep *host = nullptr; int wj = 0;
        for (size_t j = 0; j < window.size(); ++j) if (window[j].macro == W) { host = &window[j]; wj = (int)j; }
        if (host && wj == 0) { SwPlan::Batch b; b.off = c.host.size(); b.n = 0; b.macro = W; b.kind = 4; b.roff = c.rhost.size(); b.rn = 0; c.batches.push_back(b); }
        for (int kind = 0; kind < 4; ++kind) {
            items.clear(); rows.clear();
            int n_act = 0;
            for (int l = 0; l < L; ++l) { const int t = W - 1 - l; if (t >= 0 && t < T) ++n_act; }
            if (n_act == 0) continue;
            if (host) n_act += (int)host->guests.size();
            const int kz = kind == 1 ? kz_hr() : kz_ff2();
            const bool split = needs_rows(kind, n_act);
            auto problem = [&](int l, int t, const int *run_flag) {
                const size_t r0 = (size_t)t * m;
                GemmArgs g = kind == 0 ? args_gates(l, r0, m, GATES_ALL) : kind == 1 ? args_whr(l, r0, m) : kind == 2 ? args_ff1(l, r0, m) : args_ff2(l, r0, m);
                if (kind == 0 && cfg_.precision == 0) g.tile_ok = gates_tile_rows((long)m * n_act) ? 2 : 0;
                if (run_flag) { g.run_flag = run_flag; g.run_gen = 1; }
                if (split) {
                    float *ws = ws_ + r0 * d.d_model;
                    rows.push_back(row_form(g, ws, ws_mstride_, gemm_partials(m, d.d_model, kz, n_act, tk)));
                    g = partial_form(g, ws, ws_mstride_);
                } else if (tk == 2) g.force_fullk = 0;
                items.push_back(g);
            };
            for (int l = 0; l < L; ++l) {
                const int t = W - 1 - l;
                if (t < 0 || t >= T) continue;
                problem(l, t, ramp && W <= RAMP_R ? &ramp_d_->head_live[par] : nullptr);
            }
            if (host) {
                select_parity(1 - par);
                for (const auto &lt : host->guests) problem(lt.first, lt.second, &ramp_d_->guest_live[par][wj][lt.second]);
                select_parity(par);
            }
            std::vector<int> groups;
            {
                int left = (int)items.size();
                const bool cut = kind == 0 && cfg_.precision == 0 && left >= 4 && !gates_tile_rows((long)m * n_act) && lm_gates_split_on();
                while (cut && left > 0) { const int take = (left == 4 || left == 2) ? 2 : (left >= 3 ? 3 : left); groups.push_back(take); left -= take; }
                if (groups.empty()) groups.push_back((int)items.size());
            }
            size_t first = 0;
            for (size_t gi = 0; gi < groups.size(); ++gi) {
                const int gn = groups[gi];
                if (kind == 0 && !ramp && gclk_ && gclk_slots_ && gclk_used_ < GCLK_SLOTS) {
                    p.stamp_slots.push_back(std::make_pair(gclk_used_, (long)m * gn)); p.stamp_n.push_back(gn);
                    for (int i = 0; i < gn; ++i) items[first + (size_t)i].stamp = gclk_slots_ + (size_t)gclk_used_ * STAMP_WORDS;
                    ++gclk_used_;
                } else if (kind == 0 && !ramp && gclk_ && gclk_slots_ && !gclk_warned_) {
                    gclk_warned_ = true; LOGW("engine: the gates clock is out of stamp slots (%d): the gates launches of further plans are not timed", GCLK_SLOTS);
                }
                SwPlan::Batch b; b.off = c.host.size(); b.n = gn; b.macro = W; b.kind = kind; b.roff = c.rhost.size(); b.rn = gi == 0 ? (int)rows.size() : 0;
                c.host.resize(c.host.size() + (size_t)gn);
                stage_gemm_z(items.data() + first, gn, c.host.data() + b.off);
                if (gi == 0) c.rhost.insert(c.rhost.end(), rows.begin(), rows.end());
                c.batches.push_back(b);
                first += (size_t)gn;
            }
        }
    }
    m_touched();
    c.dev = dmalloc<GemmArgs>(c.host.size());
    HIP_CHECK(hipMemcpyAsync(c.dev, c.host.data(), c.host.size() * sizeof(GemmArgs), hipMemcpyHostToDevice, stream_));
    if (!c.rhost.empty()) {
        c.rdev = dmalloc<RowArgs>(c.rhost.size());
        HIP_CHECK(hipMemcpyAsync(c.rdev, c.rhost.data(), c.rhost.size() * sizeof(RowArgs), hipMemcpyHostToDevice, stream_));
    }
}

void Engine::free_sw_plans()
{
    if (!sw_plans_.empty()) LOGI("engine: feed wavefront plans emptied (%zu plans)", sw_plans_.size());
    for (auto &p : sw_plans_) for (SwPlan::Chain *c : {&p.second.one, &p.second.split}) { if (c->dev) (void)hipFree(c->dev); if (c->rdev) (void)hipFree(c->rdev); }
    sw_graphs_.clear(); sw_plans_.clear();
}

void Engine::run_sw_chain(int m, int T, bool dump_logits, const SwPlan &p, int part, hipStream_t st)
{
    const NetDims &d = L_.dims;
    const int MB = cfg_.max_batch;
    if (part < 0 || part == 0) {
        launch_advance(advance_args(m, T), st);
        encoder_front(0, m * T, step_d_ + 3 * MB, nullptr, st, part == 0 ? ws_fe_ : ws_);
    }
    if (part < 0 || part == 1) {
        static const int cls_of[4] = {T_GATES, T_GEMM_OTHER, T_GEMM_OTHER, T_GEMM_OTHER};
        const SwPlan::Chain &c = p.layers(part == 1);
        for (size_t bi = 0; bi < c.batches.size(); ++bi) {
            const SwPlan::Batch &b = c.batches[bi];
            if (b.kind == 4) { launch_ramp_latch(ramp_d_, flight_parity_, m, st); continue; }
            timed_begin(cls_of[b.kind]); launch_gemm_z(c.host.data() + b.off, b.n, c.dev + b.off, st); timed_end(cls_of[b.kind]);
            if (b.rn > 0) { timed_begin(T_ROW); launch_row_z(c.rhost.data() + b.roff, b.rn, c.rdev + b.roff, st); timed_end(T_ROW); }
        }
        if (part < 0) lm_stage_proj(m, 0, T, st, ws_);
    }
    if (part < 0 || part == 2) {
        if (part == 2) lm_stage_proj(m, 0, T, st, ws_sr_);
        hipStream_t keep = search_stream_;
        search_stream_ = st;
        for (int t = 0; t < T; ++t) run_greedy_rounds(m, dump_logits, t, eout_lm_ + (size_t)t * m * d.joiner);
        search_stream_ = keep;
    }
}

int Engine::lm_step(int m, int T, const int *slots, const int *ring_tails, const int *now_ms, float *logits_out, int mode)
{
    const int rows = m * T;
    if (m <= 0 || T <= 0 || rows > cfg_.max_batch || !flight_has_room(rows + m, 1)) { LOGE("engine: layer-major step %d x %d does not fit (max batch %d)", m, T, cfg_.max_batch); abort(); }
    HIP_CHECK(hipSetDevice(cfg_.device));
    const NetDims &d = L_.dims;
    if (!p_lm_) {
        p_lm_ = dmalloc<float>((size_t)cfg_.max_batch * 4 * d.hidden);
        for (int p = 0; p < 2; ++p) eout_lm_buf_[p] = dmalloc<float>((size_t)cfg_.max_batch * d.joiner);
        eout_lm_ = eout_lm_buf_[flight_parity_];
    }
    if (!lm_stream_) {
        HIP_CHECK(hipStreamCreateWithFlags(&lm_stream_, hipStreamNonBlocking));
        for (int i = 0; i < 9; ++i) { hipEvent_t e; HIP_CHECK(hipEventCreateWithFlags(&e, hipEventDisableTiming)); lm_events_.push_back(e); }
        for (int i = 0; i < 3; ++i) HIP_CHECK(hipEventCreateWithFlags(&zargs_done_[i], hipEventDisableTiming));
        lm_now_d_ = dmalloc<int>((size_t)cfg_.max_batch); lm_rows_d_ = dmalloc<int>((size_t)cfg_.max_batch); lm_rec_off_d_ = dmalloc<int>(1);
    }
    const int k = stage_step(m, T, slots, ring_tails, now_ms);
    std::lock_guard<std::mutex> cg(capture_mu_);
    mode == 1 ? run_feed_wavefront(m, T, logits_out != nullptr) : run_layer_major(m, T, logits_out != nullptr);
    if (logits_out) read_back_logits(k, rows, logits_out);
    return k;
}

void Engine::run_feed_wavefront(int m, int T, bool dump_logits)
{
    sw_plan(m, T);
    const bool graphs = use_graphs_ && !profiling_ && !dump_logits && (sw_graphs_.find(sw_key(m, T)) || sw_graphs_.find(sw_key(m, T, 1)) || sw_graphs_.use(m, T) >= 2);
    const bool split = graphs && split_streams_ > 0 && overlap_hint_ && flight_steps_ == 1 && !gclk_;
    const hipStream_t on[3] = {split_streams_ >= 2 ? f_stream_ : stream_, stream_, s_stream_};
    if (graphs && !sw_graphs_.find(sw_key(m, T, split ? 1 : 0)))
        capture_both_parities([&]() {
            const SwPlan &pl = sw_plan(m, T);
            if (split) for (int part = 0; part < 3; ++part) cached_graph(sw_graphs_, sw_key(m, T, 1 + part), on[part], [&]() { run_sw_chain(m, T, false, pl, part, on[part]); });
            else cached_graph(sw_graphs_, sw_key(m, T), stream_, [&]() { run_sw_chain(m, T, false, pl, -1, stream_); });
        });
    if (split) { launch_split_feed(m, T, on[0]); return; }
    general_prologue();
    if (graphs) { HIP_CHECK(hipGraphLaunch(sw_graphs_.find(sw_key(m, T)), stream_)); return; }
    launch_count_ = 0; run_sw_chain(m, T, dump_logits, sw_plan(m, T), -1, stream_); kernels_per_step_ = (launch_count_ + 1 + T - 1) / T;
}

void Engine::launch_split_feed(int m, int T, hipStream_t fe)
{
    if (fe == f_stream_) {
        if (m_unseen_by_f_) { join(f_stream_, stream_); m_unseen_by_f_ = false; }
    } else if (f_unseen_by_m_) { join(stream_, f_stream_); f_unseen_by_m_ = false; }
    if (m_unseen_by_s_) { join(s_stream_, stream_); m_unseen_by_s_ = false; }
    StreamTrace *tr = trace_slot();
    auto part = [&](int i, hipStream_t st) {
        if (tr) HIP_CHECK(hipEventRecord(tr->ev[2 * i], st));
        HIP_CHECK(hipGraphLaunch(sw_graphs_.find(sw_key(m, T, 1 + i)), st));
        if (tr) HIP_CHECK(hipEventRecord(tr->ev[2 * i + 1], st));
    };
    part(0, fe);
    if (ramp_mode_ != 0) {
        const bool hostable = ramp_mode_ == 1 && fe == f_stream_ && m_quiet_.load(std::memory_order_acquire);
        if (hostable) ramp_eligible_.fetch_add(1, std::memory_order_relaxed);
        launch_ramp_ready(ramp_d_, flight_parity_, m, T, hostable ? 1 : 0, fe);
    }
    if (fe == f_stream_) { join(stream_, f_stream_); f_unseen_by_m_ = false; }
    part(1, stream_);
    if (ramp_mode_ != 0) m_quiet_.store(true, std::memory_order_release);
    join(s_stream_, stream_); part(2, s_stream_);
    if (tr) { tr->m = m; tr->T = T; tr->used = true; }
    s_unseen_by_m_ = true; flight_tail_s_ = true;
    if (fe != f_stream_) m_unseen_by_f_ = true;
}

void Engine::run_layer_major(int m, int T, bool dump_logits)
{
    general_prologue();
    const NetDims &d = L_.dims; const int tk = f16_tile_ ? 2 : tile_ok();
    const bool wavefront = lm_wavefront_on() && !profiling_ && T > LM_WAVEFRONT_MIN_CHUNKS &&
                           gemm_fullk(m, d.d_model, kz_hr(), true, 1, tk) && gemm_fullk(m, d.d_model, kz_ff2(), true, 1, tk);
    if (wavefront) { run_lm_wavefront(m, T, dump_logits); return; }
    if (!use_graphs_ || profiling_ || dump_logits) { launch_count_ = 0; run_lm_chain(m, T, dump_logits); kernels_per_step_ = launch_count_ + 1; return; }
    const GraphCache::Key key = graph_key(m, T);
    if (!lm_graphs_.find(key) && lm_graphs_.full()) { sync(); lm_graphs_.clear(); }
    HIP_CHECK(hipGraphLaunch(cached_graph(lm_graphs_, key, stream_, [&]() { run_lm_chain(m, T, false); }), stream_));
}

int Engine::stage_step(int m, int T, const int *slots, const int *ring_tails, const int *now_ms)
{
    const size_t rows = (size_t)m * (size_t)std::max(T, 1);
    const int k = next_step_index(); int *blk = ring_h_ + ring_pos_;
    memcpy(blk, slots, (size_t)m * 4); memcpy(blk + m, ring_tails, rows * 4); memcpy(blk + m + rows, now_ms, rows * 4);
    for (int t = 0; t < T; ++t) memcpy(blk + m + 2 * rows + (size_t)t * m, slots, (size_t)m * 4);
    step_off_h_[k] = (int)ring_pos_; rec_off_h_[k] = (int)rec_pos_;
    ring_pos_ += (size_t)m + (T ? 3 : 2) * rows; rec_pos_ += 3 * rows;
    if (conf_k_h_) note_conf_step(k, slots, m, 3 * rows);
    return k;
}

void Engine::read_back_logits(int k, int rows, float *out)
{
    const size_t n = (size_t)3 * rows * L_.dims.vocab;
    HIP_CHECK(hipMemcpyAsync(logits_h_, logits_, n * 4, hipMemcpyDeviceToHost, stream_));
    HIP_CHECK(hipMemcpyAsync(rec_h_ + rec_off_h_[k], rec_d_ + rec_off_h_[k], (size_t)3 * rows * sizeof(StepRecord), hipMemcpyDeviceToHost, stream_));
    sync();
    memcpy(out, logits_h_, n * 4);
}

void Engine::apply_confidence_pending()
{
    std::vector<std::pair<int, int>> todo;
    { std::lock_guard<std::mutex> g(conf_mu_); todo.swap(conf_pending_); conf_has_pending_.store(false, std::memory_order_release); }
    if (!conf_k_h_) {
        bool any = false;
        for (const auto &t : todo) any = any || t.second > 0;
        if (!any) return;
        std::lock_guard<std::mutex> cg(capture_mu_);
        HipLegacyLock legacy;
        sync();
        drop_graphs();
        const size_t S = (size_t)cfg_.max_slots;
        conf_k_d_ = dmalloc<uint8_t>(S); conf_k_h_ = hmalloc<uint8_t>(S);
        memset(conf_k_h_, 0, S);
        conf_d_ = dmalloc<ConfRecord>(2 * rec_cap_); conf_h_ = hmalloc<ConfRecord>(2 * rec_cap_);
        LOGI("engine: confidences on (side ring %.0f MB on the device and pinned)", 2.0 * rec_cap_ * sizeof(ConfRecord) / 1e6);
    }
    for (const auto &t : todo) if (t.first >= 0 && t.first < cfg_.max_slots) conf_k_h_[t.first] = (uint8_t)t.second;
    std::lock_guard<std::mutex> cg(capture_mu_);
    m_touched();
    HIP_CHECK(hipMemcpyAsync(conf_k_d_, conf_k_h_, (size_t)cfg_.max_slots, hipMemcpyHostToDevice, stream_));
}

void Engine::drop_graphs()
{
    for (GraphCache *c : {&step_graphs_, &lm_graphs_, &lm_search_graphs_, &sw_graphs_}) c->clear();
}

BiasDesc Engine::upload_bias(const BiasSet &set, void **dev, hipStream_t st)
{
    auto pad = [](size_t b) { return (b + 15) & ~(size_t)15; };
    const size_t ns = set.state_off.size() * 4, ne = std::max<size_t>(set.edge_tok.size(), 1) * 4;
    char *p = nullptr;
    HIP_CHECK(hipMalloc((void **)&p, pad(ns) + 3 * pad(ne)));
    BiasDesc d;
    d.state_off = (const int32_t *)p; d.edge_tok = (const int32_t *)(p + pad(ns)); d.edge_next = (const int32_t *)(p + pad(ns) + pad(ne));
    d.edge_bonus = (const float *)(p + pad(ns) + 2 * pad(ne)); d.n_states = set.states(); d.flags = (int32_t)set.flags;
    HIP_CHECK(hipMemcpyAsync((void *)d.state_off, set.state_off.data(), ns, hipMemcpyHostToDevice, st));
    if (!set.edge_tok.empty()) {
        const size_t b = set.edge_tok.size() * 4;
        HIP_CHECK(hipMemcpyAsync((void *)d.edge_tok, set.edge_tok.data(), b, hipMemcpyHostToDevice, st));
        HIP_CHECK(hipMemcpyAsync((void *)d.edge_next, set.edge_next.data(), b, hipMemcpyHostToDevice, st));
        HIP_CHECK(hipMemcpyAsync((void *)d.edge_bonus, set.edge_bonus.data(), b, hipMemcpyHostToDevice, st));
    }
    *dev = p;
    return d;
}

void Engine::apply_bias_pending()
{
    std::lock_guard<std::mutex> bg(bias_mu_);
    std::vector<std::pair<int, int>> todo;
    todo.swap(bias_pending_);
    bias_has_pending_.store(false, std::memory_order_release);
    std::lock_guard<std::mutex> cg(capture_mu_);
    m_touched();
    if (!bias_set_h_) {
        bool any = false;
        for (const auto &t : todo) any = any || t.second >= 0;
        if (!any) return;
        HipLegacyLock legacy;
        sync();
        drop_graphs();
        const size_t S = (size_t)cfg_.max_slots;
        bias_set_d_ = dmalloc<int32_t>(S); bias_set_h_ = hmalloc<int32_t>(S); bias_state_d_ = dmalloc<int32_t>(S);
        bias_desc_d_ = dmalloc<BiasDesc>(kBiasSets); bias_desc_h_ = hmalloc<BiasDesc>(kBiasSets);
        for (size_t i = 0; i < S; ++i) bias_set_h_[i] = -1;
        for (int i = 0; i < kBiasSets; ++i) bias_desc_h_[i] = BiasDesc();
        HIP_CHECK(hipMemsetAsync(bias_state_d_, 0, S * 4, stream_));
        LOGI("engine: phrase boosting on");
    }
    bool tables = false;
    for (int i = 0; i < kBiasSets; ++i) {
        BiasEntry &b = bias_sets_[(size_t)i];
        if (b.set && b.users > 0 && !b.dev) {
            HipLegacyLock legacy;
            bias_desc_h_[i] = upload_bias(*b.set, &b.dev, stream_);
            HIP_CHECK(hipStreamSynchronize(stream_));
            tables = true;
        } else if (b.set && b.users == 0) {
            if (b.dev) { HipLegacyLock legacy; sync_streams(); (void)hipFree(b.dev); b.dev = nullptr; }
            bias_desc_h_[i] = BiasDesc();
            b.set.reset();
            tables = true;
        }
    }
    for (const auto &t : todo) {
        bias_set_h_[t.first] = t.second;
        HIP_CHECK(hipMemsetAsync(bias_state_d_ + t.first, 0, 4, stream_));
    }
    if (tables) HIP_CHECK(hipMemcpyAsync(bias_desc_d_, bias_desc_h_, sizeof(BiasDesc) * kBiasSets, hipMemcpyHostToDevice, stream_));
    HIP_CHECK(hipMemcpyAsync(bias_set_d_, bias_set_h_, (size_t)cfg_.max_slots * 4, hipMemcpyHostToDevice, stream_));
}

void Engine::apply_search_options_pending()
{
    std::vector<std::pair<int, SearchOpt>> todo;
    { std::lock_guard<std::mutex> g(opt_mu_); todo.swap(opt_pending_); opt_has_pending_.store(false, std::memory_order_release); }
    if (!opt_h_) {
        bool any = false;
        for (const auto &t : todo) any = any || t.second.endpoint_ms != 0;
        if (!any) return;
        std::lock_guard<std::mutex> cg(capture_mu_);
        HipLegacyLock legacy;
        sync();
        drop_graphs();
        const size_t S = (size_t)cfg_.max_slots;
        opt_d_ = dmalloc<SearchOpt>(S); opt_h_ = hmalloc<SearchOpt>(S);
        memset(opt_h_, 0, S * sizeof(SearchOpt));
        LOGI("engine: search options on");
    }
    for (const auto &t : todo) if (t.first >= 0 && t.first < cfg_.max_slots) opt_h_[t.first] = t.second;
    std::lock_guard<std::mutex> cg(capture_mu_);
    m_touched();
    HIP_CHECK(hipMemcpyAsync(opt_d_, opt_h_, (size_t)cfg_.max_slots * sizeof(SearchOpt), hipMemcpyHostToDevice, stream_));
}

int Engine::read_bias_state(int slot)
{
    if (!bias_ever_.load(std::memory_order_relaxed)) return 0;
    std::lock_guard<std::mutex> bg(bias_mu_);
    for (const auto &t : bias_pending_) if (t.first == slot) return 0;
    HipLegacyLock legacy;
    HIP_CHECK(hipSetDevice(cfg_.device));
    sync_streams();
    int v = 0;
    if (bias_state_d_) HIP_CHECK(hipMemcpy(&v, bias_state_d_ + slot, 4, hipMemcpyDeviceToHost));
    return v;
}

void Engine::note_conf_step(int k, const int *slots, int m, size_t records)
{
    bool any = false;
    for (int i = 0; i < m && !any; ++i) any = conf_k_h_[slots[i]] != 0;
    if (!any) return;
    const size_t first = (size_t)rec_off_h_[k];
    if (!conf_spans_.empty() && conf_spans_.back().first + conf_spans_.back().second == first) conf_spans_.back().second += records;
    else conf_spans_.push_back(std::make_pair(first, records));
}

void Engine::select_parity(int p)
{
    flight_parity_ = p;
    xb_ = xb_buf_[p]; u_ = u_buf_[p]; ff_ = ff_buf_[p]; xb16_ = xb16_buf_[p]; u16_ = u16_buf_[p]; ff16_ = ff16_buf_[p];
    y_ = y_buf_[p]; ssq_ = ssq_buf_[p]; y16_ = y16_buf_[p]; step_d_ = step_buf_[p]; flags_d_ = flags_buf_[p]; rec_off_d_ = rec_off_buf_[p]; eout_lm_ = eout_lm_buf_[p];
}

void Engine::begin_flight()
{
    HIP_CHECK(hipSetDevice(cfg_.device));
    const int p = flight_parity_ = next_parity_; next_parity_ ^= 1;
    if (flight_open_[p]) { HIP_CHECK(hipEventSynchronize(flight_done_[p])); flight_open_[p] = false; }
    if (conf_has_pending_.load(std::memory_order_acquire)) apply_confidence_pending();
    if (bias_has_pending_.load(std::memory_order_acquire)) apply_bias_pending();
    if (opt_has_pending_.load(std::memory_order_acquire)) apply_search_options_pending();
    conf_spans_.clear();
    ring_base_ = (size_t)p * ring_cap_; rec_base_ = (size_t)p * rec_cap_;
    ring_pos_ = ring_base_; rec_pos_ = rec_base_; flight_steps_ = 0;
    select_parity(p);
    flight_tail_s_ = false;
    { std::lock_guard<std::mutex> g(slot_mu_); zero_pending_slots(); }
}

bool Engine::flight_has_room(int rows, int nsteps) const
{
    return flight_steps_ + nsteps <= step_cap_ && ring_pos_ + (size_t)3 * rows + (size_t)cfg_.max_slots <= ring_base_ + ring_cap_ && rec_pos_ + (size_t)3 * rows <= rec_base_ + rec_cap_;
}

int Engine::step(int m, const int *slots, const int *ring_tails, const int *now_ms, float *logits_out)
{
    if (m <= 0 || m > cfg_.max_batch || !flight_has_room(m, 1)) { LOGE("engine: step of %d rows does not fit (max batch %d)", m, cfg_.max_batch); abort(); }
    const int k = stage_step(m, 0, slots, ring_tails, now_ms);
    std::lock_guard<std::mutex> cg(capture_mu_);
    general_prologue();
    const GraphCache::Key key = graph_key(m);
    if (use_graphs_ && !profiling_ && !logits_out && (step_graphs_.find(key) || step_graphs_.use(m) >= 2)) {
        if (!step_graphs_.find(key)) {
            if (step_graphs_.full()) { sync(); step_graphs_.clear(); }
            capture_both_parities([&]() { cached_graph(step_graphs_, graph_key(m), stream_, [&]() { run_chain(m, false); }); });
        }
        HIP_CHECK(hipGraphLaunch(step_graphs_.find(key), stream_));
        return k;
    }
    launch_count_ = 0; run_chain(m, logits_out != nullptr); kernels_per_step_ = launch_count_ + 1;
    if (logits_out) read_back_logits(k, m, logits_out);
    return k;
}

void Engine::decode_rows(int n, const int *slots, int op)
{
    if (n <= 0) return;
    if (dec_table_ && op == 0) return;
    HIP_CHECK(hipSetDevice(cfg_.device));
    const NetDims &d = L_.dims;
    const int MB = cfg_.max_batch;
    std::lock_guard<std::mutex> cg(capture_mu_);
    general_prologue();
    for (int o = 0; o < n; o += MB) {
        const int m = std::min(MB, n - o);
        if (ring_pos_ + (size_t)m > ring_base_ + ring_cap_) { LOGE("engine: index ring exhausted"); abort(); }
        int *blk = ring_h_ + ring_pos_;
        memcpy(blk, slots + o, (size_t)m * 4);
        ring_pos_ += (size_t)m;
        HIP_CHECK(hipMemcpyAsync(dec_slots_d_, blk, (size_t)m * 4, hipMemcpyHostToDevice, stream_));
        DecRowsArgs a; a.slot_idx = dec_slots_d_; a.M = m; a.op = op; a.blank = P_.blank_id; a.state = gstate_; a.dec = dec_params(); a.de_out = dec_table_ ? nullptr : de_; a.ld_de = d.d_model;
        a.bias_state = bias_state_d_;
        timed_begin(T_DEC); launch_dec_rows(a, stream_); timed_end(T_DEC);
        if (!dec_table_) run_decproj(m, dec_slots_d_, nullptr, nullptr, 1);
    }
}

int Engine::close_flight()
{
    HIP_CHECK(hipSetDevice(cfg_.device));
    std::lock_guard<std::mutex> cg(capture_mu_);
    hipStream_t tail = s_stream_;
    if (!(flight_tail_s_ && s_unseen_by_m_)) {
        tail = stream_;
        if (f_unseen_by_m_) { join(stream_, f_stream_); f_unseen_by_m_ = false; }
        if (s_unseen_by_m_) { join(stream_, s_stream_); s_unseen_by_m_ = false; }
    }
    if (rec_pos_ > rec_base_) HIP_CHECK(hipMemcpyAsync(rec_h_ + rec_base_, rec_d_ + rec_base_, (rec_pos_ - rec_base_) * sizeof(StepRecord), hipMemcpyDeviceToHost, tail));
    for (const auto &sp : conf_spans_) {
        HIP_CHECK(hipMemcpyAsync(conf_h_ + sp.first, conf_d_ + sp.first, sp.second * sizeof(ConfRecord), hipMemcpyDeviceToHost, tail));
        conf_copied_.fetch_add(sp.second, std::memory_order_relaxed);
    }
    conf_spans_.clear();
    HIP_CHECK(hipEventRecord(flight_done_[flight_parity_], tail));
    flight_open_[flight_parity_] = true;
    return flight_parity_;
}

bool Engine::flight_done(int parity)
{
    const hipError_t e = hipEventQuery(flight_done_[parity]);
    if (e == hipSuccess) return true;
    if (e != hipErrorNotReady) HIP_CHECK(e);
    (void)hipGetLastError();
    return false;
}

void Engine::wait_flight(int parity)
{
    HIP_CHECK(hipSetDevice(cfg_.device));
    HIP_CHECK(hipEventSynchronize(flight_done_[parity]));
    if (profiling_) sync();
}

void Engine::end_flight() { wait_flight(close_flight()); }

void Engine::zero_slots(int n)
{
    const NetDims &d = L_.dims;
    for (int i = 0; i < n; ++i) {
        ZeroSlotArgs z;
        z.h = h_; z.c = c_; z.n_layers = d.n_layers; z.slots = (size_t)cfg_.max_slots; z.d_model = d.d_model; z.hidden = d.hidden;
        z.eout = eout_; z.dout = dout_; z.joiner = d.joiner; z.state = gstate_; z.blank = P_.blank_id; z.slot = i; z.h16 = h16_;
        launch_zero_slot(z, stream_);
    }
    HIP_CHECK(hipStreamSynchronize(stream_));
}

void Engine::debug_encoder(int n, const float *x, const float *h, const float *c, float *eout, float *h2, float *c2)
// ... 308 lines not shown
```

### april_asr_amd/csrc/engine.h

```cpp
#pragma once
#include <hip/hip_runtime.h>
#include <atomic>
#include <cstdint>
#include <deque>
#include <array>
#include <functional>
#include <map>
#include <memory>
#include <mutex>
#include <string>
#include <utility>
#include <vector>
#include "bias.h"
#include "fbank_tables.h"
#include "resample.h"
#include "input_format.h"
#include "kernels.h"
#include "host_pool.h"
#include "model_loader.h"

namespace aprilx {

struct PackedLayout {
    NetDims dims;
    size_t conv_w[3], conv_b[3];
    int k3 = 0;
    size_t w_embed, b_embed;
    struct Layer { size_t wg, bg, whr, wff1, bff1, wff2, bff2; };
    std::vector<Layer> layers;
    size_t w_encproj, b_encproj, emb, dec_conv, dec_conv_b, w_decproj, b_decproj, w_out, b_out;
    size_t total = 0;
    int vocab_pad = 0;
    bool has_dec_conv_b = false;
    std::vector<float> norm_eps;
    float embed_eps = 0;
};
void plan_layout(const NetDims &d, bool has_dec_conv_b, PackedLayout &L);
std::vector<std::pair<size_t, size_t>> gemm_sections(const PackedLayout &L);
void pack_weights(const HostModel &m, PackedLayout &L, std::vector<float> &blob);

std::recursive_mutex &hip_legacy_mutex();
struct HipLegacyLock { std::lock_guard<std::recursive_mutex> g; HipLegacyLock() : g(hip_legacy_mutex()) {} };

struct EngineConfig {
    int device = 0;
    int max_slots = 4096;
    int max_batch = 2048;
    int precision = 0;
};

struct KernelTiming { double ms = 0; long launches = 0; };

struct GraphCache {
    using Key = std::array<int, 3>;
    const char *name; size_t cap;
    bool full() const { return map_.size() >= cap; }
    hipGraphExec_t find(const Key &k) const { auto it = map_.find(k); return it == map_.end() ? nullptr : it->second; }
    void insert(const Key &k, hipGraphExec_t g) { map_[k] = g; }
    int use(int m, int T = 0) { return ++uses_[std::make_pair(m, T)]; }
    void clear();
    std::map<Key, hipGraphExec_t> map_; std::map<std::pair<int, int>, int> uses_;
};

struct RampStep { int macro = 0, own = 0; std::vector<std::pair<int, int>> guests; };
std::vector<RampStep> ramp_window(int L, int T, int R, int max_problems = 3);

class Engine {
public:
    Engine(const EngineConfig &cfg, const PackedLayout &layout, const float *blob_host, const float *blob_device,
           const ModelParams &params, const FbankHostTables &ft, const std::vector<uint8_t> &tok_class);
    ~Engine();

    int device() const { return cfg_.device; }
    int max_batch() const { return cfg_.max_batch; }
    int max_slots() const { return cfg_.max_slots; }
    int ring_frames() const { return ring_frames_; }
    const NetDims &dims() const { return L_.dims; }
    hipStream_t stream() const { return stream_; }
    const float *weights_device() const { return w_; }
    float *weights_mut() { return w_; }
    void finish_weights();
    int precision() const { return cfg_.precision; }
    int tile_ok() const { return cfg_.precision == 0 ? 1 : 0; }
    bool f16_tile() const { return f16_tile_; }
    const PackedLayout &layout() const { return L_; }

    int alloc_slot();
    void free_slot(int slot);
    int live_slots() const { return live_.load(std::memory_order_relaxed); }

    void fbank(int n_frames, const FbankFrameDesc *desc, const std::pair<const int16_t *, size_t> *parts, size_t n_parts, size_t n_pcm,
               HostPool *pool = nullptr);
    void set_resample_pass(int n, ResampleDesc *rs, const ResampleSpec *const *specs, const std::pair<const int16_t *, size_t> *in_parts,
                           size_t n_in_parts, size_t n_in)
    {
        rs_n_ = n; rs_desc_ = rs; rs_specs_ = specs; rs_in_parts_ = in_parts; rs_n_in_parts_ = n_in_parts; rs_n_in_ = n_in;
    }
    void set_decode_pass(int n, const DecodeDesc *dc, const std::pair<const uint8_t *, size_t> *raw_parts, size_t n_raw_parts, size_t n_raw)
    {
        dc_n_ = n; dc_desc_ = dc; dc_raw_parts_ = raw_parts; dc_n_raw_parts_ = n_raw_parts; dc_n_raw_ = n_raw;
    }
    void decode_counts(uint64_t *launches, uint64_t *frames) const
    {
        *launches = dc_launches_.load(std::memory_order_relaxed); *frames = dc_frames_.load(std::memory_order_relaxed);
    }
    void begin_flight();
    bool flight_has_room(int rows, int nsteps = 1) const;
    int step(int m, const int *slots, const int *ring_tails, const int *now_ms, float *logits_out = nullptr);
    int lm_step(int m, int T, const int *slots, const int *ring_tails, const int *now_ms, float *logits_out = nullptr, int mode = 0);
    int lm_max_rows() const { return cfg_.max_batch; }
    void decode_rows(int n, const int *slots, int op);
    int close_flight();
    bool flight_done(int parity);
    void wait_flight(int parity);
    void end_flight();
    bool profiling() const { return profiling_; }
    void set_overlap_hint(bool on) { overlap_hint_ = on; }
    const StepRecord *records(int step_index) const { return rec_h_ + rec_off_h_[step_index]; }
    void set_slot_confidence(int slot, int k)
    {
        std::lock_guard<std::mutex> g(conf_mu_);
        conf_pending_.push_back(std::make_pair(slot, k));
        if (k > 0) conf_ever_.store(true, std::memory_order_relaxed);
        conf_has_pending_.store(true, std::memory_order_release);
    }
    const ConfRecord *conf_records(int step_index) const { return conf_h_ ? conf_h_ + rec_off_h_[step_index] : nullptr; }
    uint64_t confidence_records() const { return conf_copied_.load(std::memory_order_relaxed); }
    static constexpr int kBiasSets = 64;
    bool set_slot_bias(int slot, const std::shared_ptr<const BiasSet> &set)
    {
        std::lock_guard<std::mutex> g(bias_mu_);
        if (slot < 0 || slot >= cfg_.max_slots) return false;
        if (bias_slot_set_.empty()) {
            if (!set) return true;
            bias_slot_set_.assign((size_t)cfg_.max_slots, -1); bias_sets_.resize(kBiasSets);
        }
        int idx = -1;
        if (set) {
            if (set->vocab != L_.dims.vocab || set->vocab > kBiasMaxVocab) return false;
            for (int i = 0; i < kBiasSets && idx < 0; ++i) if (bias_sets_[(size_t)i].set == set) idx = i;
            for (int i = 0; i < kBiasSets && idx < 0; ++i) if (!bias_sets_[(size_t)i].set) idx = i;
            if (idx < 0) return false;
            bias_sets_[(size_t)idx].set = set;
            ++bias_sets_[(size_t)idx].users;
        }
        const int old = bias_slot_set_[(size_t)slot];
        if (old < 0 && idx < 0) return true;
        if (old >= 0) --bias_sets_[(size_t)old].users;
        bias_slot_set_[(size_t)slot] = idx;
        bias_pending_.push_back(std::make_pair(slot, idx));
        if (set) bias_ever_.store(true, std::memory_order_relaxed);
        bias_has_pending_.store(true, std::memory_order_release);
        return true;
    }
    int read_bias_state(int slot);
    void debug_decide_biased(int n, int op, const float *logits, float early_emit, const int *now_ms, int round, int32_t *state_io, StepRecord *rec_out,
                             const BiasSet &set, int32_t *bias_state_io);
    void set_slot_search_options(int slot, SearchOpt o)
    {
        std::lock_guard<std::mutex> g(opt_mu_);
        if (o.endpoint_ms == 0 && !opt_ever_.load(std::memory_order_relaxed)) return;
        opt_pending_.push_back(std::make_pair(slot, o));
        if (o.endpoint_ms) opt_ever_.store(true, std::memory_order_relaxed);
        opt_has_pending_.store(true, std::memory_order_release);
    }
    void debug_decide_opts(int n, int op, const float *logits, float early_emit, const int *now_ms, int round, int32_t *state_io, StepRecord *rec_out,
                           const BiasSet *set, int32_t *bias_state_io, const SearchOpt *opts);
    void sync();
    void sync_streams();

    void debug_encoder(int n, const float *x, const float *h, const float *c, float *eout, float *h2, float *c2);
    void debug_decoder(int n, const int64_t *ctx, float *dout);
    void debug_joiner(int n, const float *eout, const float *dout, float *logits);
    void debug_decide(int n, int op, const float *logits, float early_emit, const int *now_ms, int round, int32_t *state_io, StepRecord *rec_out);
    void debug_confidence(int n, const float *logits, int k, ConfRecord *out, const BiasSet *set = nullptr, const int32_t *bias_state = nullptr);
    void debug_fbank(int n_frames, const int16_t *pcm_frames , float *out );
    void debug_resample(const ResampleSpec *spec, const int16_t *pcm, size_t n, int16_t *out);
    void debug_decode(uint32_t encoding, uint32_t channels, int32_t channel, const void *data, size_t n_frames, int16_t *out);
    void read_ring(int slot, int row, int n_rows, float *out);
    void read_greedy_state(int slot, GreedyState *out);

    void set_profiling(bool on);
    void set_gates_clock(bool on);
    void gates_clock(double *ms, long *launches, long *rows) const { *ms = gclk_ms_; *launches = gclk_launches_; *rows = gclk_rows_; }
    void gates_clock_by_n(double *ms4, long *launches4) const { for (int i = 0; i < 4; ++i) { ms4[i] = gclk_ms_n_[i]; launches4[i] = gclk_launches_n_[i]; } }
    KernelTiming timing(int cls) const { return timing_[cls]; }
    void ramp_counts(uint64_t *hosted, uint64_t *eligible);
    void reset_timing();
    enum { T_GATES = 0, T_GEMM_OTHER = 1, T_ROW = 2, T_CONV = 3, T_FBANK = 4, T_DEC = 5, T_RESAMPLE = 6, T_DECODE = 7, T_COUNT = 8 };
    long kernels_per_step() const { return kernels_per_step_.load(std::memory_order_relaxed); }

private:
    void upload_tables(const FbankHostTables &ft);
    void zero_slots(int n);
    void run_encoder_rows(int n, const float *x_direct);
    void encoder_front(size_t r0, int rows, const int *row_slots, const float *x_direct, hipStream_t st, float *ws);
    void lm_stage_layer(int l, int m, int t0, int t1, hipStream_t st);
    void lm_stage_proj(int m, int t0, int t1, hipStream_t st, float *ws);
    enum { GATES_ALL = 0xF, GATES_X = 0x3, GATES_H = 0xC };
    RowScale in_scale(int l, size_t r0) const;
    GemmArgs args_gates(int l, size_t r0, int rows, int waves) const;
    GemmArgs args_whr(int l, size_t r0, int rows) const;
    GemmArgs args_ff1(int l, size_t r0, int rows) const;
    GemmArgs args_ff2(int l, size_t r0, int rows) const;
    GemmArgs args_encproj(size_t r0, int rows, const int *slot_idx, float *out) const;
    AdvanceArgs advance_args(int m, int T) const;
    struct GreedyIo {
        int gen = 1;
        const int *now = nullptr;
        const float *eout = nullptr;
        const int *eout_rows = nullptr;
        const int *rec_off = nullptr; int rec_slot0 = 0;
        float *dump = nullptr;
    };
    void run_greedy_rounds(int n, bool dump_logits, int chunk = 0, const float *eout_rows = nullptr);
    void run_greedy_rounds(int n, const GreedyIo &io);
    void run_lm_chain(int m, int T, bool dump_logits);
    void run_lm_wavefront(int m, int T, bool dump_logits);
    struct SwPlan {
        struct Batch { size_t off; int n, macro, kind; size_t roff; int rn; };
        struct Chain { std::vector<GemmArgs> host; GemmArgs *dev = nullptr; std::vector<Batch> batches; std::vector<RowArgs> rhost; RowArgs *rdev = nullptr; };
        Chain one;
        Chain split;
        bool hosts = false;
        const Chain &layers(bool split_feed) const { return split_feed && !split.batches.empty() ? split : one; }
        std::vector<std::pair<int, long>> stamp_slots; std::vector<int> stamp_n;
    };
    GraphCache::Key graph_key(int m, int T = 0, int part = 0) const { return {m, T, flight_parity_ * 4 + part}; }
    GraphCache::Key sw_key(int m, int T, int part = 0) const { return graph_key(gclk_ ? -m : m, T, part); }
    SwPlan &sw_plan(int m, int T);
    void build_sw_chain(SwPlan &p, SwPlan::Chain &c, int m, int T, bool ramp);
    void free_sw_plans();
    void run_sw_chain(int m, int T, bool dump_logits, const SwPlan &p, int part, hipStream_t st);
    int stage_step(int m, int T, const int *slots, const int *ring_tails, const int *now_ms); void read_back_logits(int k, int rows, float *out);
    template <typename Chain> hipGraphExec_t cached_graph(GraphCache &cache, const GraphCache::Key &key, hipStream_t st, Chain &&chain);
    template <typename Capture> void capture_both_parities(Capture &&capture);
    void run_feed_wavefront(int m, int T, bool dump_logits); void run_layer_major(int m, int T, bool dump_logits); void launch_split_feed(int m, int T, hipStream_t fe);
    struct StreamTrace { hipEvent_t ev[6] = {nullptr, nullptr, nullptr, nullptr, nullptr, nullptr}; int m = 0, T = 0; bool used = false; };
    std::deque<StreamTrace> trace_; hipEvent_t trace_base_ = nullptr;
    StreamTrace *trace_slot();
    void dump_stream_trace();
    void select_parity(int p);
    void join(hipStream_t waiter, hipStream_t src);
    void general_prologue();
    int next_step_index() { ++flight_steps_; return (int)(step_seq_++ & (uint64_t)(2 * step_cap_ - 1)); }
    void launch_rowepi(GemmArgs fused_form, float *ws, hipStream_t st, bool force = false, int cls = T_GEMM_OTHER);
    bool gates_tile_rows(long rows) const;
    void run_decproj(int n, const int *d_slots, const int *row_mask, const int *run_flag, int run_gen, float *out = nullptr);
    void build_dec_table();
    void run_chain(int m, bool dump_logits);
    void collect_gates_clock();
    void timed_begin(int cls);
    void timed_end(int cls);
    void collect_timing();
    DecEmbedParams dec_params() const;

    EngineConfig cfg_;
    PackedLayout L_;
    ModelParams P_;
    hipStream_t stream_ = nullptr;
    float *w_ = nullptr;
    uint16_t *wh_ = nullptr;
    void lin(GemmArgs &g, size_t off) const { if (wh_) { g.wp = wh_ + off; g.wt = 1; } else { g.wp = w_ + off; g.wt = 0; } }
    bool f16_tile_ = false;
    uint16_t *wx_ = nullptr;
    uint16_t *y16_ = nullptr, *xb16_ = nullptr, *u16_ = nullptr, *ff16_ = nullptr;
    uint16_t *h16_ = nullptr;
    int kzx_hr_ = 1, kzx_ff2_ = 1;
    void lin16(GemmArgs &g, size_t off) const { g.wp = wx_ + off; g.wt = 1; g.tile_ok = 2; }
    int kz_hr() const { return f16_tile_ ? kzx_hr_ : kz_hr_; }
    int kz_ff2() const { return f16_tile_ ? kzx_ff2_ : kz_ff2_; }
    float *h_ = nullptr, *c_ = nullptr, *ring_ = nullptr, *eout_ = nullptr, *dout_ = nullptr;
    GreedyState *gstate_ = nullptr;
    float *dec_table_ = nullptr;
    uint8_t *cls_ = nullptr;
    int ring_frames_ = 0;
    float *xin_ = nullptr, *a3_ = nullptr, *y_ = nullptr, *ssq_ = nullptr, *xb_ = nullptr, *u_ = nullptr, *ff_ = nullptr, *ws_ = nullptr, *ws_g_ = nullptr, *de_ = nullptr;
    float *logits_ = nullptr;
    float *p_lm_ = nullptr, *eout_lm_ = nullptr;
    int *ring_h_ = nullptr; size_t ring_cap_ = 0, ring_pos_ = 0;
    int *step_off_h_ = nullptr, *rec_off_h_ = nullptr; int step_cap_ = 0;
    StepRecord *rec_d_ = nullptr, *rec_h_ = nullptr; size_t rec_cap_ = 0, rec_pos_ = 0;
    int flight_parity_ = 0, next_parity_ = 0; size_t ring_base_ = 0, rec_base_ = 0; int flight_steps_ = 0;
    uint64_t step_seq_ = 0;
    hipEvent_t flight_done_[2] = {nullptr, nullptr};
    std::mutex conf_mu_;
    std::vector<std::pair<int, int>> conf_pending_;
    std::atomic<bool> conf_has_pending_{false}, conf_ever_{false};
    uint8_t *conf_k_d_ = nullptr, *conf_k_h_ = nullptr;
    ConfRecord *conf_d_ = nullptr, *conf_h_ = nullptr;
    std::vector<std::pair<size_t, size_t>> conf_spans_;
    std::atomic<uint64_t> conf_copied_{0};
    void apply_confidence_pending();
    void drop_graphs();
    struct BiasEntry { std::shared_ptr<const BiasSet> set; int users = 0; void *dev = nullptr; };
    std::mutex bias_mu_;
    std::vector<BiasEntry> bias_sets_;
    std::vector<int> bias_slot_set_;
    std::vector<std::pair<int, int>> bias_pending_;
    std::atomic<bool> bias_has_pending_{false}, bias_ever_{false};
    int32_t *bias_set_d_ = nullptr, *bias_set_h_ = nullptr, *bias_state_d_ = nullptr;
    BiasDesc *bias_desc_d_ = nullptr, *bias_desc_h_ = nullptr;
    void apply_bias_pending();
    std::mutex opt_mu_;
    std::vector<std::pair<int, SearchOpt>> opt_pending_;
    std::atomic<bool> opt_has_pending_{false}, opt_ever_{false};
    SearchOpt *opt_d_ = nullptr, *opt_h_ = nullptr;
    void apply_search_options_pending();
    BiasDesc upload_bias(const BiasSet &set, void **dev, hipStream_t st);
    void debug_decide_impl(int n, int op, const float *logits, float early_emit, const int *now_ms, int round, int32_t *state_io, StepRecord *rec_out,
                           const BiasSet *set, int32_t *bias_state_io, const SearchOpt *opts = nullptr);
    void note_conf_step(int k, const int *slots, int m, size_t records);
    bool flight_open_[2] = {false, false};
    hipStream_t f_stream_ = nullptr, s_stream_ = nullptr, search_stream_ = nullptr;
    std::vector<hipEvent_t> join_ev_; size_t join_pos_ = 0;
    bool f_unseen_by_m_ = false, s_unseen_by_m_ = false, m_unseen_by_f_ = false, m_unseen_by_s_ = false, flight_tail_s_ = false;
    bool overlap_hint_ = false;
    int split_streams_ = 2;
    int ramp_mode_ = 1;
    RampState *ramp_d_ = nullptr;
    std::atomic<bool> m_quiet_{false};
    void m_touched() { m_quiet_.store(false, std::memory_order_release); }
    std::atomic<uint64_t> ramp_eligible_{0};
    float *xb_buf_[2] = {nullptr, nullptr}, *u_buf_[2] = {nullptr, nullptr}, *ff_buf_[2] = {nullptr, nullptr};
    uint16_t *xb16_buf_[2] = {nullptr, nullptr}, *u16_buf_[2] = {nullptr, nullptr}, *ff16_buf_[2] = {nullptr, nullptr};
    float *y_buf_[2] = {nullptr, nullptr}, *ssq_buf_[2] = {nullptr, nullptr}, *eout_lm_buf_[2] = {nullptr, nullptr}, *ws_fe_ = nullptr, *ws_sr_ = nullptr;
    uint16_t *y16_buf_[2] = {nullptr, nullptr};
    int *step_buf_[2] = {nullptr, nullptr}, *flags_buf_[2] = {nullptr, nullptr}, *rec_off_buf_[2] = {nullptr, nullptr};
    int *counter_d_ = nullptr, *step_d_ = nullptr, *active_d_ = nullptr, *dirty_d_ = nullptr, *rec_off_d_ = nullptr, *flags_d_ = nullptr;
    int *dec_slots_d_ = nullptr;
    float *logits_h_ = nullptr;
    FbankFrameDesc *hs_desc_[2] = {nullptr, nullptr}, *ds_desc_[2] = {nullptr, nullptr}; int desc_cap_ = 0;
    int16_t *hs_pcm_[2] = {nullptr, nullptr}, *ds_pcm_[2] = {nullptr, nullptr}; size_t pcm_cap_ = 0;
    int fb_flip_ = 0;
    hipEvent_t fb_done_[2] = {nullptr, nullptr};
    std::vector<size_t> part_off_;
    size_t rs_cap_ = 0;
    int rs_n_ = 0;
    ResampleDesc *rs_desc_ = nullptr;
    const ResampleSpec *const *rs_specs_ = nullptr;
    const std::pair<const int16_t *, size_t> *rs_in_parts_ = nullptr;
    size_t rs_n_in_parts_ = 0, rs_n_in_ = 0;
    size_t dc_cap_ = 0;
    int dc_n_ = 0;
    const DecodeDesc *dc_desc_ = nullptr;
    const std::pair<const uint8_t *, size_t> *dc_raw_parts_ = nullptr;
    size_t dc_n_raw_parts_ = 0, dc_n_raw_ = 0;
    std::atomic<uint64_t> dc_launches_{0}, dc_frames_{0};
    std::mutex rs_mu_;
    std::map<const ResampleSpec *, const float *> rs_tables_;
    const float *resample_table(const ResampleSpec *spec);
    FbankTables ft_;
    std::vector<void *> table_allocs_;
    float pad_value_ = 0;
    std::vector<int> free_, zero_pending_;
    void zero_pending_slots();
    std::atomic<int> live_{0};
    std::mutex slot_mu_;
    std::mutex capture_mu_;
    int kz_embed_ = 1, kz_hr_ = 1, kz_ff2_ = 1, kz_proj_ = 1, kz_out_ = 1;
    int ws_mstride_ = 0;
    float *conv_wt_ = nullptr;
    bool use_graphs_ = true;
    GraphCache step_graphs_{"chunk step", 256};
    GraphCache lm_graphs_{"layer-major chain", 32};
    GraphCache lm_search_graphs_{"long-feed search", 64};
    GraphCache sw_graphs_{"feed wavefront", 4 * 64};
    size_t sw_plan_cap_ = 64;
    std::map<GraphCache::Key, SwPlan> sw_plans_;
    hipStream_t lm_stream_ = nullptr;
    std::vector<hipEvent_t> lm_events_;
    GemmArgs *zargs_h_ = nullptr, *zargs_d_ = nullptr; size_t zargs_region_ = 0, zargs_pos_ = 0;
    hipEvent_t zargs_done_[3] = {nullptr, nullptr, nullptr}; bool zargs_busy_[3] = {false, false, false}; int zargs_next_ = 0;
    int *lm_now_d_ = nullptr, *lm_rows_d_ = nullptr, *lm_rec_off_d_ = nullptr;
    std::atomic<long> kernels_per_step_{0};
    long launch_count_ = 0;
    bool profiling_ = false;
    bool gclk_ = false, gclk_warned_ = false; unsigned long long *gclk_slots_ = nullptr; int gclk_used_ = 0;
    static constexpr int GCLK_SLOTS = 2048;
    double gclk_ms_ = 0; long gclk_launches_ = 0, gclk_rows_ = 0; double gclk_ms_n_[4] = {0, 0, 0, 0}; long gclk_launches_n_[4] = {0, 0, 0, 0};
    struct Ev { hipEvent_t a, b; int cls; };
    std::vector<Ev> ev_pool_; size_t ev_used_ = 0;
    KernelTiming timing_[T_COUNT];
};

}
```

### april_asr_amd/csrc/kernels.h

```cpp
#pragma once
#include <hip/hip_runtime.h>
#include <cstdint>

namespace aprilx {

enum GemmEpilogue {
    EPI_PARTIAL = 0,
    EPI_LSTM = 1,
    EPI_BIAS_DSWISH = 2,
    EPI_HR = 3,
    EPI_RESID_SSQ = 4,
    EPI_SLOT_STORE = 5,
    EPI_XPART = 6
};
enum GemmAOp { AOP_NONE = 0, AOP_TANH_ADD = 1 };
enum GemmMode { GM_SLAB = 0, GM_FULLK = 1, GM_TILE = 2, GM_KW = 3, GM_PP = 4 };


constexpr int SSQ_COLS = 32;

struct RowScale {
    const float *ssq = nullptr;
    int groups = 0;
    float inv_n = 0.0f;
    float eps = 0.0f;
};

struct GreedyState { int32_t ctx0, ctx1; int32_t last_tok; uint32_t last_emit_ms; };

constexpr int STAMP_WORDS = 144, STAMP_ENDS = 8, STAMP_NENDS = 64, STAMP_SUBS = 72;

struct GemmArgs {
    const float *a0 = nullptr; int lda0 = 0; const int *aidx0 = nullptr; int K0 = 0;
    const float *a1 = nullptr; int lda1 = 0; const int *aidx1 = nullptr; int K1 = 0;
    const float *a0b = nullptr;
    const int *aidx0b = nullptr; int same_idx_b = 1;
    const GreedyState *ctx_state = nullptr; int ctx_vocab = 0;
    int a_op = AOP_NONE;
    RowScale x_scale;
    const void *wp = nullptr;
    int wt = 0;
    int M = 0, N = 0, K = 0;
    int kz = 1;
    int zs = 1;
    int mode = GM_SLAB;
    int epi = EPI_PARTIAL;
    float *out = nullptr; int ldo = 0;
    void *out16 = nullptr;
    void *state16 = nullptr;
    int m_stride = 0;
    const float *bias = nullptr;
    float *c_state = nullptr;
    const int *slot_idx = nullptr;
    int hidden = 0;
    float *state = nullptr; int ld_state = 0;
    const float *resid = nullptr; int ldr = 0;
    RowScale r_scale;
    float *ssq_out = nullptr;
    const int *row_mask = nullptr;
    const int *run_flag = nullptr;
    int run_gen = 1;
    int wave_mask = 0xF;
    const float *p_add = nullptr; int ldp = 0;
    int force_fullk = 0;
    int zcount = 1;
    int tile_ok = 0;
    int asm_loop = 0;
    unsigned long long *trace = nullptr;
    unsigned long long *stamp = nullptr;
    int debug = 0;
};
void launch_gemm(const GemmArgs &g, hipStream_t s);
void gemm_profile_next_launch(hipEvent_t start, hipEvent_t stop);
bool gemm_profile_pending();
void launch_gemm_tile(const GemmArgs &g, int mt, int nt, const GemmArgs *dev_args, int n, hipStream_t s);
int gemm_kw_waves(const GemmArgs &g);
bool gemm_pp_ok(const GemmArgs &g, int mt);
void launch_gemm_pp(const GemmArgs &g, int mt, const GemmArgs *dev_args, int n, hipStream_t s);
bool gemm_pw_ok(const GemmArgs &g);
void launch_gemm_pw(const GemmArgs &g, const GemmArgs *dev_args, int n, hipStream_t s);
void gemm_pp_pin(int enable, int mt);
bool gemm_kw_has_kernel(const GemmArgs &g, int mt, int nt);
void launch_gemm_kw(const GemmArgs &g, int mt, int nt, const GemmArgs *dev_args, int n, hipStream_t s);
void gemm_kw_pin(int enable, int mt);
int recur_form(const GemmArgs &g);
void launch_recur(const GemmArgs &g, int form, const GemmArgs *dev_args, int n, hipStream_t s);
void stage_gemm_z(const GemmArgs *items, int n, GemmArgs *staged);
void launch_gemm_z(const GemmArgs *staged, int n, const GemmArgs *dev_args, hipStream_t s);
int gemm_partials(int M, int N, int kz, int zcount = 1, int tile_ok = 0);
bool gemm_fullk(int M, int N, int kz, bool force = false, int zcount = 1, int tile_ok = 0);
bool gemm_tile_planned(int M, int N, int kz, int zcount = 1);
void gemm_tile_pin(int enable, int mt, int zs);

enum RowMode {
    ROW_HR = 0,
    ROW_RESID_SSQ = 1,
    ROW_SLOT_STORE = 2
};
struct RowArgs {
    int mode = ROW_HR;
    const float *ws = nullptr; int parts = 1; int m_stride = 0; int N = 0; int M = 0;
    const float *bias = nullptr;
    const float *resid = nullptr; int ldr = 0;
    RowScale r_scale;
    float *out = nullptr; int ldo = 0;
    const int *slot_idx = nullptr;
    float *state = nullptr; int ld_state = 0;
    float *ssq_out = nullptr;
    void *out16 = nullptr, *state16 = nullptr;
    const int *row_mask = nullptr;
    const int *run_flag = nullptr;
    int run_gen = 1;
};
void launch_row(const RowArgs &r, hipStream_t s);
void launch_row_z(const RowArgs *host_args, int n, const RowArgs *dev_args, hipStream_t s);

constexpr int RAMP_R = 2;
struct RampState {
    unsigned long long ready[2];
    int head_live[2];
    int guest_live[2][RAMP_R][RAMP_R];
    unsigned generation;
    unsigned hosted;
};
constexpr int RAMP_MAX_M = 0xFFFFF, RAMP_MAX_T = 0xFF;
void launch_ramp_ready(RampState *rs, int q, int m, int T, int hostable, hipStream_t s);
void launch_ramp_latch(RampState *rs, int p, int m, hipStream_t s);

struct StepRecord { int32_t idx; float max_val; float blank_val; uint32_t flags; };
constexpr int kConfMaxAlt = 8;
struct ConfRecord { float lse; float blank_val; int32_t n_alt; uint32_t reserved; int32_t alt_id[kConfMaxAlt]; float alt_logit[kConfMaxAlt]; };
static_assert(sizeof(ConfRecord) == 80, "ConfRecord is 20 x 32 bit");
enum { REC_VALID = 1, REC_BLANK = 2, REC_CTX = 4 };
enum TokClassBits { TKC_WORD_START = 1, TKC_SENT_END = 2, TKC_COMMA = 4, TKC_DOT = 8, TKC_DIGIT_START = 16 };

struct BiasDesc { const int32_t *state_off = nullptr, *edge_tok = nullptr, *edge_next = nullptr; const float *edge_bonus = nullptr; int32_t n_states = 0, flags = 0; };

struct SearchOpt { uint32_t endpoint_ms; float blank_penalty; };
static_assert(sizeof(SearchOpt) == 8, "SearchOpt is 2 x 32 bit");

struct DecEmbedParams {
    const float *emb = nullptr;
    const float *conv_w = nullptr;
    const float *conv_b = nullptr;
    int d = 0, groups = 0, context = 0, vocab = 0;
};

struct DecideArgs {
    const float *ws = nullptr; int parts = 1; int m_stride = 0; int N = 0; int M = 0;
    int n_valid = 0;
    const float *bias = nullptr;
    int blank = 0;
    float early_emit = 0.0f;
    const int *slot_idx = nullptr;
    const int *now_ms = nullptr;
    int *active = nullptr;
    int gen = 1;
    int rec_slot = 0;
    int *dirty = nullptr;
    const uint8_t *tok_class = nullptr;
    GreedyState *state = nullptr;
    StepRecord *rec = nullptr;
    StepRecord *rec_ring = nullptr;
    const int *rec_off = nullptr; int round = 0;
    float *logits_dump = nullptr;
    DecEmbedParams dec;
    float *de_out = nullptr; int ld_de = 0;
    int *run_flags = nullptr;
    int *rerun_flags = nullptr;
    const uint8_t *conf_k = nullptr;
    ConfRecord *conf_ring = nullptr;
    ConfRecord *conf = nullptr; int conf_k_all = 0;
    const int32_t *bias_set = nullptr;
    int32_t *bias_state = nullptr;
    const BiasDesc *bias_desc = nullptr;
    const SearchOpt *opt = nullptr;
};
void launch_decide(const DecideArgs &a, hipStream_t s);

struct DecRowsArgs {
    const int *slot_idx = nullptr; int M = 0;
    int op = 0; int blank = 0;
    GreedyState *state = nullptr;
    DecEmbedParams dec;
    float *de_out = nullptr; int ld_de = 0;
    int32_t *bias_state = nullptr;
};
void launch_dec_rows(const DecRowsArgs &a, hipStream_t s);

struct DecEmbedArgs {
    DecEmbedParams dec;
    const int *ctx = nullptr;
    int M = 0;
    float *out = nullptr; int ldo = 0;
};
void launch_dec_embed(const DecEmbedArgs &a, hipStream_t s);

struct AdvanceArgs {
    const int *host_ring = nullptr;
    const int *host_step_off = nullptr;
    const int *host_rec_off = nullptr;
    int *counter = nullptr;
    int index_mask = 0x7fffffff;
    int *dst = nullptr; int dst_stride = 0;
    int n_arrays = 3; int len[4] = {0, 0, 0, 0};
    int *rec_off = nullptr;
    int *flags = nullptr; int n_flags = 0;
};
void launch_advance(const AdvanceArgs &a, hipStream_t s);

struct ZeroSlotArgs {
    float *h = nullptr, *c = nullptr; int n_layers = 0; size_t slots = 0; int d_model = 0, hidden = 0;
    float *eout = nullptr, *dout = nullptr; int joiner = 0;
    GreedyState *state = nullptr; int blank = 0;
    int slot = 0;
    void *h16 = nullptr;
    int n_list = 0; int list[64] = {0};
};
void launch_zero_slot(const ZeroSlotArgs &a, hipStream_t s);

struct BlockSetupArgs {
    const int *now_src = nullptr; int *now_dst = nullptr;
    int *rows_dst = nullptr; int row0 = 0; int count = 0;
    const int *rec_off_step = nullptr; int *rec_off_block = nullptr; int rec_add = 0;
    int *flags = nullptr; int n_flags = 0;
};
void launch_block_setup(const BlockSetupArgs &a, hipStream_t s);

struct ConvEmbedArgs {
    const float *ring = nullptr;
    int ring_frames = 0, mel = 0, seg = 0;
    const int *slot_idx = nullptr;
    const int *ring_tail = nullptr;
    const float *w[3] = {nullptr, nullptr, nullptr};
    const float *b[3] = {nullptr, nullptr, nullptr};
    int ch[3] = {0, 0, 0};
    int ch1_per_group = 0;
    int stride[3] = {1, 2, 2};
    float *out = nullptr; int ldo = 0;
    int M = 0;
    const float *x_direct = nullptr;
    const float *w0t = nullptr, *w1t = nullptr;
};
void launch_conv_embed(const ConvEmbedArgs &a, hipStream_t s);
void launch_conv_weight_transpose(const float *w0, const float *w1, int c0, int c1, float *w0t, float *w1t, hipStream_t s);

void launch_cvt_f16(const float *src, void *dst, size_t n, hipStream_t s);

void launch_repack_x32(const float *src_packed, void *dst, int K, int N, hipStream_t s);

struct FbankTables {
    const float *window = nullptr;
    const double *tw[16] = {nullptr};
    const double *tws[16] = {nullptr};
    int fct[16] = {0}; int nfct = 0;
    const float *mel = nullptr;
    const int *mel_lo = nullptr;
    const int *mel_hi = nullptr;
    int padded = 0, nbins = 0;
};
struct FbankFrameDesc { int32_t slot; int32_t ring_row; int32_t pcm_off; };
struct FbankArgs {
    FbankTables t;
    const int16_t *pcm = nullptr;
    const FbankFrameDesc *desc = nullptr;
    int n_frames = 0;
    float *ring = nullptr; int ring_frames = 0;
    float pad_value = 0.0f;
};
void launch_fbank(const FbankArgs &a, hipStream_t s);

struct ResampleDesc {
    const float *taps = nullptr;
    int64_t in_base = 0;
    int64_t out_first = 0;
    int64_t out_end = 0;
    int32_t in_off = 0, in_n = 0;
    int32_t out_dst = 0, out_cnt = 0;
    int32_t L = 1, M = 1, K = 0, ldt = 0;
};
struct ResampleArgs {
    const int16_t *in = nullptr;
    int16_t *out = nullptr;
    const ResampleDesc *desc = nullptr;
    int n_desc = 0;
    int max_blocks = 0;
    int lds_floats = 0;
};
void launch_resample(const ResampleArgs &a, hipStream_t s);

constexpr int kDecodeBlock = 256;
struct DecodeDesc {
    int64_t src_off = 0;
    int32_t dst = 0;
    int32_t out_cnt = 0, n_src = 0;
    uint8_t encoding = 0, channels = 1; int8_t channel = 0;
    uint8_t dst_in = 0;
};
struct DecodeArgs {
    const uint8_t *raw = nullptr;
    int16_t *out = nullptr;
    const DecodeDesc *desc = nullptr;
    int n_desc = 0;
    int max_blocks = 0;
};
void launch_decode(const DecodeArgs &a, hipStream_t s);

}
```

### april_asr_amd/csrc/kernels_misc.hip

```cpp
#include "kernels.h"
#include "device_utils.h"
#include "env.h"
#include <algorithm>
#include <cstdio>
#include <cstdlib>

namespace aprilx {

template <int MODE>
__device__ __forceinline__ void row_body(const RowArgs &r)
{
    if (r.run_flag && *r.run_flag != r.run_gen) return;
    const int m = blockIdx.x;
    const int tid = threadIdx.x;
    const int slot = r.slot_idx ? r.slot_idx[m] : m;
    if (MODE == ROW_SLOT_STORE) { if (r.row_mask && !r.row_mask[m]) return; }
    float rs = 1.0f;
    const bool scaled = MODE == ROW_HR || (MODE == ROW_SLOT_STORE && r.r_scale.ssq != nullptr);
    if (scaled) rs = row_scale(r.r_scale, m);
    const int nq = r.N >> 2;
    for (int q0 = 0; q0 < nq; q0 += 256) {
        const int q = q0 + tid;
        const bool ok = q < nq;
        const int n = q * 4;
        f32x4 s = f32x4{0.f, 0.f, 0.f, 0.f};
        if (ok) s = tree_sum4(r.ws, r.parts, r.m_stride, r.N, m, n);
        if (MODE == ROW_HR) {
            if (ok) {
                const HrTail t = hr_tail(s, *reinterpret_cast<const f32x4 *>(r.resid + (size_t)m * r.ldr + n), rs);
                *reinterpret_cast<f32x4 *>(r.state + (size_t)slot * r.ld_state + n) = t.state;
                *reinterpret_cast<f32x4 *>(r.out + (size_t)m * r.ldo + n) = t.out;
                if (r.state16) *reinterpret_cast<h4 *>(reinterpret_cast<_Float16 *>(r.state16) + (size_t)slot * r.ld_state + n) = to_h4(t.state);
                if (r.out16) *reinterpret_cast<h4 *>(reinterpret_cast<_Float16 *>(r.out16) + (size_t)m * r.ldo + n) = to_h4(t.out);
            }
        } else if (MODE == ROW_RESID_SSQ) {
            f32x4 y = f32x4{0.f, 0.f, 0.f, 0.f};
            if (ok) {
                const f32x4 res = r.resid ? *reinterpret_cast<const f32x4 *>(r.resid + (size_t)m * r.ldr + n) : f32x4{0.f, 0.f, 0.f, 0.f};
                y = resid_tail(s, *reinterpret_cast<const f32x4 *>(r.bias + n), res, r.resid != nullptr);
                *reinterpret_cast<f32x4 *>(r.out + (size_t)m * r.ldo + n) = y;
                if (r.out16) *reinterpret_cast<h4 *>(reinterpret_cast<_Float16 *>(r.out16) + (size_t)m * r.ldo + n) = to_h4(y);
            }
            float ss;
            if (granule_ssq_store(y, ok, q, ss)) r.ssq_out[(size_t)m * (r.N / SSQ_COLS) + n / SSQ_COLS] = ss;
        } else {
            if (ok) {
                const f32x4 b = *reinterpret_cast<const f32x4 *>(r.bias + n);
                *reinterpret_cast<f32x4 *>(r.out + (size_t)slot * r.ldo + n) = scaled ? slot_value(s, rs, b) : slot_value(s, b);
            }
        }
    }
}

template <int MODE>
__global__ __launch_bounds__(256) void row_kernel(RowArgs r) { row_body<MODE>(r); }

template <int MODE>
__global__ __launch_bounds__(256) void row_zkernel(const RowArgs *__restrict__ zargs)
{
    const RowArgs r = zargs[blockIdx.y];
    row_body<MODE>(r);
}

void launch_row(const RowArgs &r, hipStream_t s)
{
    dim3 grid((unsigned)r.M), block(256);
    switch (r.mode) {
    case ROW_HR: hipLaunchKernelGGL(row_kernel<ROW_HR>, grid, block, 0, s, r); break;
    case ROW_RESID_SSQ: hipLaunchKernelGGL(row_kernel<ROW_RESID_SSQ>, grid, block, 0, s, r); break;
    default: hipLaunchKernelGGL(row_kernel<ROW_SLOT_STORE>, grid, block, 0, s, r); break;
    }
}

void launch_row_z(const RowArgs *host_args, int n, const RowArgs *dev_args, hipStream_t s)
{
    if (n <= 0) return;
    const RowArgs &r = host_args[0];
    for (int i = 1; i < n; ++i)
        if (host_args[i].mode != r.mode || host_args[i].M != r.M || host_args[i].N != r.N || host_args[i].parts != r.parts) {
            fprintf(stderr, "libapril(mi355x): launch_row_z: the problems of one launch must have one shape\n"); abort();
        }
    dim3 grid((unsigned)r.M, (unsigned)n), block(256);
    switch (r.mode) {
    case ROW_HR: hipLaunchKernelGGL(row_zkernel<ROW_HR>, grid, block, 0, s, dev_args); break;
    case ROW_RESID_SSQ: hipLaunchKernelGGL(row_zkernel<ROW_RESID_SSQ>, grid, block, 0, s, dev_args); break;
    default: hipLaunchKernelGGL(row_zkernel<ROW_SLOT_STORE>, grid, block, 0, s, dev_args); break;
    }
}

__global__ __launch_bounds__(64) void ramp_ready_kernel(RampState *rs, int q, int m, int T, int hostable)
{
    if (threadIdx.x != 0) return;
    __hip_atomic_store(&rs->head_live[q], 1, __ATOMIC_RELAXED, __HIP_MEMORY_SCOPE_AGENT);
    const unsigned g = __hip_atomic_load(&rs->generation, __ATOMIC_RELAXED, __HIP_MEMORY_SCOPE_AGENT) + 1u;
    __hip_atomic_store(&rs->generation, g, __ATOMIC_RELAXED, __HIP_MEMORY_SCOPE_AGENT);
    __builtin_amdgcn_fence(__ATOMIC_RELEASE, "agent");
    asm volatile("s_waitcnt vmcnt(0)" ::: "memory");
    const unsigned long long rec = ((unsigned long long)g << 32) | ((unsigned long long)(unsigned)m << 12) | ((unsigned long long)(unsigned)T << 4) | (unsigned long long)(hostable & 1);
    __hip_atomic_store(&rs->ready[q], rec, __ATOMIC_RELAXED, __HIP_MEMORY_SCOPE_AGENT);
}

__global__ __launch_bounds__(64) void ramp_latch_kernel(RampState *rs, int p, int m)
{
    if (threadIdx.x != 0) return;
    const unsigned long long mine = __hip_atomic_load(&rs->ready[p], __ATOMIC_RELAXED, __HIP_MEMORY_SCOPE_AGENT);
    const unsigned long long next = __hip_atomic_load(&rs->ready[1 - p], __ATOMIC_RELAXED, __HIP_MEMORY_SCOPE_AGENT);
    const unsigned g = (unsigned)(mine >> 32);
    const int next_m = (int)((next >> 12) & RAMP_MAX_M), next_T = (int)((next >> 4) & RAMP_MAX_T);
    const bool host = (unsigned)(next >> 32) == g + 1u && next_m == m && (int)((mine >> 12) & RAMP_MAX_M) == m && (next & 1ull) != 0;
    if (host) {
        __builtin_amdgcn_fence(__ATOMIC_ACQUIRE, "agent");
        __hip_atomic_store(&rs->head_live[1 - p], 0, __ATOMIC_RELAXED, __HIP_MEMORY_SCOPE_AGENT);
        rs->hosted += 1u;
    }
    for (int j = 1; j <= RAMP_R; ++j)
        for (int t = 0; t < RAMP_R; ++t) rs->guest_live[p][j - 1][t] = (host && t < j && t < next_T) ? 1 : 0;
}

void launch_ramp_ready(RampState *rs, int q, int m, int T, int hostable, hipStream_t s)
{
    hipLaunchKernelGGL(ramp_ready_kernel, dim3(1), dim3(64), 0, s, rs, q, m, T, hostable);
}
void launch_ramp_latch(RampState *rs, int p, int m, hipStream_t s)
{
    hipLaunchKernelGGL(ramp_latch_kernel, dim3(1), dim3(64), 0, s, rs, p, m);
}

__device__ __forceinline__ void dec_embed_row(const DecEmbedParams &p, int tok0, int tok1, float *out)
{
    const int cg = p.d / p.groups;
    for (int o = threadIdx.x; o < p.d; o += 256) {
        const int g0 = (o / cg) * cg;
        const float *w = p.conv_w + (size_t)o * cg * p.context;
        float acc = 0.0f;
        for (int ci = 0; ci < cg; ++ci) {
            acc += p.emb[(size_t)tok0 * p.d + g0 + ci] * w[ci * p.context + 0];
            acc += p.emb[(size_t)tok1 * p.d + g0 + ci] * w[ci * p.context + 1];
        }
        if (p.conv_b) acc += p.conv_b[o];
        out[o] = acc > 0.0f ? acc : 0.0f;
    }
}

#include "kernels_bias.inc"
#include "kernels_confidence.inc"

template <bool CONF, bool BIAS, bool OPT>
__device__ __forceinline__ void decide_body(const DecideArgs &a)
{
    extern __shared__ __attribute__((aligned(16))) unsigned char bias_lds[];
    __shared__ float s_best[4], s_blank[4];
    __shared__ int s_idx[4];
    __shared__ int s_ctx[3];
    if (a.round > 0 && a.run_flags && a.run_flags[a.round] != a.gen) return;
    const int m = blockIdx.x;
    const int tid = threadIdx.x;
    StepRecord *rec = a.rec ? a.rec + m : a.rec_ring + (size_t)a.rec_off[0] + (size_t)a.rec_slot * a.M + m;
    if (a.round > 0 && a.active[m] != a.gen) {
        if (tid == 0) { rec->idx = -1; rec->max_val = 0.0f; rec->blank_val = 0.0f; rec->flags = 0; a.dirty[m] = 0; }
        return;
    }
    float best = -9999999999.0f;
    int best_i = -1;
    float blank_v = 0.0f;
    BiasRow br;
    if (BIAS) bias_row_begin(a, m, bias_lds, br);
    if (BIAS && br.bonus) bias_scan(a, m, br, best, best_i, blank_v);
    else
    for (int n = tid; n < a.n_valid; n += 256) {
        const float v = tree_sum(a.ws, a.parts, a.m_stride, a.N, m, n) + a.bias[n];
        if (a.logits_dump) a.logits_dump[(size_t)m * a.n_valid + n] = v;
        if (n == a.blank) blank_v = v;
        else if (v > best) { best = v; best_i = n; }
    }
#pragma unroll
    for (int off = 32; off > 0; off >>= 1) {
        const float ov = __shfl_xor(best, off);
        const int oi = __shfl_xor(best_i, off);
        const bool take = (oi >= 0) && (best_i < 0 || ov > best || (ov == best && oi < best_i));
        if (take) { best = ov; best_i = oi; }
        blank_v += __shfl_xor(blank_v, off);
    }
    const int wave = tid >> 6;
    if ((tid & 63) == 0) { s_best[wave] = best; s_idx[wave] = best_i; s_blank[wave] = blank_v; }
    __syncthreads();
    if (tid == 0) {
        float b = s_best[0]; int bi = s_idx[0];
        for (int w = 1; w < 4; ++w) {
            const float ov = s_best[w]; const int oi = s_idx[w];
            if (oi >= 0 && (bi < 0 || ov > b || (ov == b && oi < bi))) { b = ov; bi = oi; }
        }
        float bl = s_blank[(a.blank & 255) >> 6];
        rec->idx = bi; rec->max_val = b; rec->blank_val = bl;

        const int slot = a.slot_idx[m];
        GreedyState st = a.state[slot];
        SearchOpt so; so.endpoint_ms = 0u; so.blank_penalty = 0.0f;
        if (OPT) { so = a.opt[slot]; if (so.endpoint_ms) bl = bl - so.blank_penalty; }
        int tok = bi; float tv = b;
        if (tok < 0) { tok = a.blank == 0 ? 1 : 0; tv = -9999999999.0f; }
        const bool cleared = st.ctx1 == a.blank;
        const bool same = st.ctx1 == tok;
        const float ee = same ? 0.0f : a.early_emit;
        bool is_blank = (bl - ee) > tv;
        const unsigned tc = a.tok_class[tok];
        bool punct = (tc & (TKC_SENT_END | TKC_COMMA)) != 0;
        if (punct && st.last_tok >= 0 && (a.tok_class[st.last_tok] & TKC_DIGIT_START) && (tc & TKC_DOT)) punct = false;
        if (!cleared && punct && !same && tv > (bl - 3.5f)) is_blank = false;
        const unsigned now = (unsigned)a.now_ms[m];
        unsigned flags = REC_VALID;
        bool rerun = false, silence = false;
        if (!is_blank) {
            st.last_emit_ms = now;
            st.ctx0 = st.ctx1; st.ctx1 = tok;
            st.last_tok = tok;
            rerun = true;
        } else {
            flags |= REC_BLANK;
            if (OPT && so.endpoint_ms) silence = now - st.last_emit_ms >= so.endpoint_ms;
            else if (now - st.last_emit_ms >= 2200u) { silence = true; }
            if (silence) {
                st.last_tok = -1;
                if (st.ctx0 != a.blank) { st.ctx0 = a.blank; st.ctx1 = a.blank; rerun = true; }
            }
        }
        a.active[m] = is_blank ? 0 : a.gen;
        if (rerun) flags |= REC_CTX;
        rec->flags = flags;
        a.state[slot] = st;
        if (BIAS && br.bonus) bias_row_end(a, br, slot, is_blank, tok, OPT ? silence : is_blank && now - st.last_emit_ms >= 2200u);
        a.dirty[m] = rerun ? 1 : 0;
        if (a.run_flags) {
            if (!is_blank && a.round < 2) a.run_flags[a.round + 1] = a.gen;
            if (rerun) a.rerun_flags[a.round] = a.gen;
        }
        s_ctx[0] = st.ctx0; s_ctx[1] = st.ctx1; s_ctx[2] = rerun ? 1 : 0;
    }
    __syncthreads();
    if (s_ctx[2] && a.de_out) dec_embed_row(a.dec, s_ctx[0], s_ctx[1], a.de_out + (size_t)m * a.ld_de);
    if (CONF) {
        if (a.conf) confidence_row(a, m, a.conf_k_all, a.conf + m, BIAS ? br.bonus : nullptr);
        else {
            const int k = a.conf_k[a.slot_idx[m]];
            if (k) confidence_row(a, m, k, a.conf_ring + (rec - a.rec_ring), BIAS ? br.bonus : nullptr);
        }
    }
}

__global__ __launch_bounds__(256) void decide_kernel(DecideArgs a) { decide_body<false, false, false>(a); }
__global__ __launch_bounds__(256) void decide_conf_kernel(DecideArgs a) { decide_body<true, false, false>(a); }
__global__ __launch_bounds__(256) void decide_bias_kernel(DecideArgs a) { decide_body<false, true, false>(a); }
__global__ __launch_bounds__(256) void decide_conf_bias_kernel(DecideArgs a) { decide_body<true, true, false>(a); }
__global__ __launch_bounds__(256) void decide_opt_kernel(DecideArgs a) { decide_body<false, false, true>(a); }
__global__ __launch_bounds__(256) void decide_conf_opt_kernel(DecideArgs a) { decide_body<true, false, true>(a); }
__global__ __launch_bounds__(256) void decide_bias_opt_kernel(DecideArgs a) { decide_body<false, true, true>(a); }
__global__ __launch_bounds__(256) void decide_conf_bias_opt_kernel(DecideArgs a) { decide_body<true, true, true>(a); }

void launch_decide(const DecideArgs &a, hipStream_t s)
{
    const bool conf = a.conf || a.conf_k;
    if (a.bias_set) {
        if (a.n_valid > 8192 || !a.bias_state || !a.bias_desc) { fprintf(stderr, "libapril(mi355x): launch_decide: phrase boosting needs a vocabulary of at most 8192 tokens and all three tables\n"); abort(); }
        const size_t lds = bias_lds_bytes(a.n_valid);
        if (a.opt) {
            if (conf) hipLaunchKernelGGL(decide_conf_bias_opt_kernel, dim3((unsigned)a.M), dim3(256), lds, s, a);
            else hipLaunchKernelGGL(decide_bias_opt_kernel, dim3((unsigned)a.M), dim3(256), lds, s, a);
        }
        else if (conf) hipLaunchKernelGGL(decide_conf_bias_kernel, dim3((unsigned)a.M), dim3(256), lds, s, a);
        else hipLaunchKernelGGL(decide_bias_kernel, dim3((unsigned)a.M), dim3(256), lds, s, a);
    }
    else if (a.opt) {
        if (conf) hipLaunchKernelGGL(decide_conf_opt_kernel, dim3((unsigned)a.M), dim3(256), 0, s, a);
        else hipLaunchKernelGGL(decide_opt_kernel, dim3((unsigned)a.M), dim3(256), 0, s, a);
    }
    else if (conf) hipLaunchKernelGGL(decide_conf_kernel, dim3((unsigned)a.M), dim3(256), 0, s, a);
    else hipLaunchKernelGGL(decide_kernel, dim3((unsigned)a.M), dim3(256), 0, s, a);
}

__global__ __launch_bounds__(256) void dec_rows_kernel(DecRowsArgs a)
{
    __shared__ int s_ctx[2];
    const int m = blockIdx.x;
    if (threadIdx.x == 0) {
        const int slot = a.slot_idx[m];
        GreedyState st = a.state[slot];
        if (a.op == 1) {
            st.last_tok = -1;
            if (st.ctx0 != a.blank) { st.ctx0 = a.blank; st.ctx1 = a.blank; }
            a.state[slot] = st;
            if (a.bias_state) a.bias_state[slot] = 0;
        }
        s_ctx[0] = st.ctx0; s_ctx[1] = st.ctx1;
    }
    __syncthreads();
    if (a.de_out) dec_embed_row(a.dec, s_ctx[0], s_ctx[1], a.de_out + (size_t)m * a.ld_de);
}

void launch_dec_rows(const DecRowsArgs &a, hipStream_t s)
{
    hipLaunchKernelGGL(dec_rows_kernel, dim3((unsigned)a.M), dim3(256), 0, s, a);
}

__global__ __launch_bounds__(256) void dec_embed_kernel(DecEmbedArgs a)
{
    const int m = blockIdx.x;
    dec_embed_row(a.dec, a.ctx[m * a.dec.context + 0], a.ctx[m * a.dec.context + 1], a.out + (size_t)m * a.ldo);
}

void launch_dec_embed(const DecEmbedArgs &a, hipStream_t s)
{
    hipLaunchKernelGGL(dec_embed_kernel, dim3((unsigned)a.M), dim3(256), 0, s, a);
}

__global__ __launch_bounds__(1024) void advance_kernel(AdvanceArgs a)
{
    __shared__ int s_k;
    if (threadIdx.x == 0) s_k = a.counter[0];
    __syncthreads();
    const int kc = s_k, k = kc & a.index_mask;
    const int *src = a.host_ring + a.host_step_off[k];
    for (int arr = 0; arr < a.n_arrays; ++arr) {
        for (int i = threadIdx.x; i < a.len[arr]; i += 1024) a.dst[arr * a.dst_stride + i] = src[i];
        src += a.len[arr];
    }
    if (threadIdx.x < a.n_flags) a.flags[threadIdx.x] = 0;
    if (threadIdx.x == 0) { a.rec_off[0] = a.host_rec_off[k]; a.counter[0] = (kc + 1) & 0x7fffffff; }
}

void launch_advance(const AdvanceArgs &a, hipStream_t s)
{
    hipLaunchKernelGGL(advance_kernel, dim3(1), dim3(1024), 0, s, a);
}

__global__ __launch_bounds__(256) void zero_slot_kernel(ZeroSlotArgs a)
{
    const int l = blockIdx.x;
    const size_t s = (size_t)(a.n_list > 0 ? a.list[blockIdx.y] : a.slot);
    if (l < a.n_layers) {
        float *h = a.h + ((size_t)l * a.slots + s) * a.d_model, *c = a.c + ((size_t)l * a.slots + s) * a.hidden;
        for (int i = threadIdx.x; i < a.d_model; i += 256) h[i] = 0.0f;
        if (a.h16) { _Float16 *hh = reinterpret_cast<_Float16 *>(a.h16) + ((size_t)l * a.slots + s) * a.d_model; for (int i = threadIdx.x; i < a.d_model; i += 256) hh[i] = (_Float16)0.0f; }
        for (int i = threadIdx.x; i < a.hidden; i += 256) c[i] = 0.0f;
    } else {
        for (int i = threadIdx.x; i < a.joiner; i += 256) { a.eout[s * a.joiner + i] = 0.0f; a.dout[s * a.joiner + i] = 0.0f; }
        if (threadIdx.x == 0) { GreedyState st; st.ctx0 = a.blank; st.ctx1 = a.blank; st.last_tok = -1; st.last_emit_ms = 0; a.state[s] = st; }
    }
}

void launch_zero_slot(const ZeroSlotArgs &a, hipStream_t s)
{
    hipLaunchKernelGGL(zero_slot_kernel, dim3((unsigned)a.n_layers + 1, (unsigned)std::max(1, a.n_list)), dim3(256), 0, s, a);
}

__global__ __launch_bounds__(256) void block_setup_kernel(BlockSetupArgs a)
{
    for (int i = threadIdx.x; i < a.count; i += 256) { a.now_dst[i] = a.now_src[i]; a.rows_dst[i] = a.row0 + i; }
    if ((int)threadIdx.x < a.n_flags) a.flags[threadIdx.x] = 0;
    if (threadIdx.x == 0) a.rec_off_block[0] = a.rec_off_step[0] + a.rec_add;
}

void launch_block_setup(const BlockSetupArgs &a, hipStream_t s)
{
    hipLaunchKernelGGL(block_setup_kernel, dim3(1), dim3(256), 0, s, a);
}

__global__ __launch_bounds__(256) void conv12_kernel(ConvEmbedArgs a)
{
    extern __shared__ __attribute__((aligned(16))) float lds[];
    const int m = blockIdx.x, grp = blockIdx.y;
    const int tid = threadIdx.x;
    const int H0 = a.seg, W0 = a.mel;
    const int s0 = a.stride[0], s1 = a.stride[1], s2 = a.stride[2];
    const int H1 = (H0 - 3) / s0 + 1, W1 = (W0 - 3) / s0 + 1;
    const int H2 = (H1 - 3) / s1 + 1, W2 = (W1 - 3) / s1 + 1;
    const int W3 = (W2 - 3) / s2 + 1;
    const int c0 = a.ch[0], cg = a.ch1_per_group;
    float *x = lds;
    float *a1 = x + H0 * W0;
    float *a2 = a1 + c0 * H1 * W1;

    if (a.x_direct) {
        for (int i = tid; i < H0 * W0; i += 256) x[i] = a.x_direct[(size_t)m * H0 * W0 + i];
    } else {
        const int slot = a.slot_idx[m];
        const int tail = a.ring_tail[m];
        const float *ring = a.ring + (size_t)slot * a.ring_frames * W0;
        for (int i = tid; i < H0 * W0; i += 256) {
            const int row = i / W0, col = i % W0;
            x[i] = ring[(size_t)((tail + row) % a.ring_frames) * W0 + col];
        }
    }
    __syncthreads();
    for (int p = tid; p < H1 * W1; p += 256) {
        const int oh = p / W1, ow = p % W1;
        float patch[9];
#pragma unroll
        for (int i = 0; i < 3; ++i)
#pragma unroll
            for (int j = 0; j < 3; ++j) patch[i * 3 + j] = x[(oh * s0 + i) * W0 + ow * s0 + j];
        for (int c = 0; c < c0; ++c) {
            const float *w = a.w[0] + c * 9;
            float acc = 0.0f;
#pragma unroll
            for (int k = 0; k < 9; ++k) acc += patch[k] * w[k];
            acc += a.b[0][c];
            a1[c * H1 * W1 + p] = dswish(acc);
        }
    }
    __syncthreads();
    {
        const int NP = H2 * W2;
        const int per = ((NP + 63) / 64) * 64;
        int nsub = per <= 256 ? 256 / per : 1;
        while (nsub > 1 && (cg % nsub) != 0) --nsub;
        const int cps = cg / nsub;
        const int stride = per <= 256 ? per : 256;
        const int sub = per <= 256 ? __builtin_amdgcn_readfirstlane(tid / per) : 0;
        for (int base = 0; base < NP; base += stride) {
            const int p = base + (per <= 256 ? tid % per : tid);
            if (sub < nsub && p < NP) {
                const int oh = p / W2, ow = p % W2;
                float acc[8];
#pragma unroll
                for (int cc = 0; cc < 8; ++cc) acc[cc] = 0.0f;
                for (int ci = 0; ci < c0; ++ci) {
                    const float *src = a1 + ci * H1 * W1 + (oh * s1) * W1 + ow * s1;
                    float patch[9];
#pragma unroll
// ... 206 lines not shown
```

Before: 20040.

## Replace device-side ramp merge with event-gated head chain on the front stream

Removes the device-flag ramp merge, where a predecessor feed hosted the next feed's head problems under run flags with latch and ready kernels. Instead, the layer wavefront plan is split into a head chain (the first macro steps), run on the F stream behind a window event recorded by the previous feed's body chain, and a body chain on M. The event sits inside the body graph when the HIP runtime can capture an external event record; otherwise it is recorded between two body sub-graphs. This drops the extra kernels and the guest GEMM problems, but adds more graph parts per shape, extra event waits and cross-stream ordering that must stay correct.

```diff
diff --git a/april_asr_amd/csrc/engine.cc b/april_asr_amd/csrc/engine.cc
--- a/april_asr_amd/csrc/engine.cc
+++ b/april_asr_amd/csrc/engine.cc
@@ -225,7 +225,19 @@
     xb_ = xb_buf_[0]; u_ = u_buf_[0]; ff_ = ff_buf_[0];
     ramp_mode_ = env_int("APRIL_RAMP_MERGE", 1);
     if (ramp_mode_ < 0 || ramp_mode_ > 2) ramp_mode_ = 1;
-    ramp_d_ = dmalloc<RampState>(1); HIP_CHECK(hipMemset(ramp_d_, 0, sizeof(RampState)));
+    for (int p = 0; p < 2; ++p) HIP_CHECK(hipEventCreateWithFlags(&window_ev_[p], hipEventDisableTiming));
+    if (ramp_mode_ != 0 && env_int("APRIL_RAMP_EVENT_NODE", 1) != 0) {
+        HipLegacyLock capture_guard;
+        hipGraph_t g = nullptr;
+        if (hipStreamBeginCapture(stream_, hipStreamCaptureModeRelaxed) == hipSuccess) {
+            const hipError_t rec = hipEventRecordWithFlags(window_ev_[0], stream_, hipEventRecordExternal);
+            const hipError_t end = hipStreamEndCapture(stream_, &g);
+            event_node_ = rec == hipSuccess && end == hipSuccess && g != nullptr;
+            if (g) (void)hipGraphDestroy(g);
+        }
+        (void)hipGetLastError();
+        LOGI("engine: ramp overlap: the window event is %s", event_node_ ? "a node of the body graph" : "recorded between two body graphs (this HIP runtime captures no external event record)");
+    }
     de_ = dmalloc<float>(MB * d.d_model);
     HIP_CHECK(hipMemset(de_, 0, MB * d.d_model * 4));
     logits_ = dmalloc<float>(3 * MB * d.vocab);
@@ -247,7 +259,7 @@
     upload_tables(ft);
     use_graphs_ = env_int("APRIL_NO_GRAPHS", 0) == 0;
     if (const int n = env_int("APRIL_GRAPH_CACHE_CAP", 0))
-        step_graphs_.cap = lm_graphs_.cap = lm_search_graphs_.cap = sw_plan_cap_ = (size_t)std::max(n, 2), sw_graphs_.cap = 4 * sw_plan_cap_;
+        step_graphs_.cap = lm_graphs_.cap = lm_search_graphs_.cap = sw_plan_cap_ = (size_t)std::max(n, 2), sw_graphs_.cap = 6 * sw_plan_cap_;
     free_.reserve(S);
     for (int i = cfg_.max_slots - 1; i >= 0; --i) free_.push_back(i);
     LOGI("engine: device %d, %d slots, max batch %d, weights %.1f MB, kz(embed,hr,ff2,proj,out)=%d,%d,%d,%d,%d",
@@ -315,10 +327,8 @@
     (void)hipSetDevice(cfg_.device);
     (void)hipStreamSynchronize(f_stream_); (void)hipStreamSynchronize(stream_); (void)hipStreamSynchronize(s_stream_);
     dump_stream_trace();
-    if (ramp_d_ && ramp_eligible_.load() > 0) {
-        unsigned h = 0;
-        if (hipMemcpy(&h, &ramp_d_->hosted, sizeof h, hipMemcpyDeviceToHost) == hipSuccess) LOGI("engine: ramp merge: %u of %llu hostable split feeds were hosted by their predecessor", h, (unsigned long long)ramp_eligible_.load());
-    }
+    if (ramp_eligible_.load() > 0) LOGI("engine: ramp overlap: the head chains of %llu split feeds ran behind their predecessor's window event", (unsigned long long)ramp_hosted_.load());
+    for (hipEvent_t e : window_ev_) if (e) (void)hipEventDestroy(e);
     for (StreamTrace &t : trace_) for (hipEvent_t e : t.ev) if (e) (void)hipEventDestroy(e);
     if (trace_base_) (void)hipEventDestroy(trace_base_);
     for (hipEvent_t e : join_ev_) (void)hipEventDestroy(e);
@@ -347,7 +357,7 @@
                         (void *)xb16_buf_[p], (void *)u16_buf_[p], (void *)ff16_buf_[p], (void *)rec_off_buf_[p], (void *)flags_buf_[p], (void *)step_buf_[p]}) if (q) (void)hipFree(q);
     if (ws_fe_) (void)hipFree(ws_fe_);
     if (ws_sr_) (void)hipFree(ws_sr_);
-    for (void *p : {(void *)wx_, (void *)h16_, (void *)ramp_d_}) if (p) (void)hipFree(p);
+    for (void *p : {(void *)wx_, (void *)h16_}) if (p) (void)hipFree(p);
     for (void *p : {(void *)w_, (void *)wh_, (void *)h_, (void *)c_, (void *)ring_, (void *)eout_, (void *)dout_, (void *)gstate_, (void *)cls_, (void *)ws_, (void *)xin_,
                     (void *)a3_, (void *)de_, (void *)logits_, (void *)rec_d_, (void *)counter_d_,
                     (void *)active_d_, (void *)dirty_d_, (void *)dec_slots_d_,
@@ -491,20 +501,23 @@
     FILE *f = fopen(path, "w");
     if (!f) return;
     fprintf(f, "# one line per split feed; times in us since the first split feed; FE = index fetch + conv + embed on stream F, LY = layer wavefront on M, SR = encoder_proj + search on S\n");
-    fprintf(f, "# feed sessions chunks  FE_start FE_end  LY_start LY_end  SR_start SR_end   overlap: FE inside the previous feed's LY window? SR inside the next feed's LY window?\n");
-    std::vector<std::array<float, 6>> ts;
+    fprintf(f, "# where the plan separates a head chain (ramp overlap), LY is the body chain on M and HD the head chain on F; HD_start is stamped behind F's wait for the window event; else HD is -1 -1\n");
+    fprintf(f, "# feed sessions chunks  FE_start FE_end  LY_start LY_end  SR_start SR_end   overlap: FE inside the previous feed's LY window? SR inside the next feed's LY window?   HD_start HD_end  offered?  HD started before the previous feed's LY end?\n");
+    struct Line { std::array<float, 8> a; int m, T; bool head, offered; };
+    std::vector<Line> ts;
     for (StreamTrace &t : trace_) {
-        std::array<float, 6> a{};
+        Line ln; ln.a.fill(-1e-3f); ln.m = t.m; ln.T = t.T; ln.head = t.head; ln.offered = t.offered;
         bool ok = t.used;
-        for (int i = 0; i < 6 && ok; ++i) ok = hipEventElapsedTime(&a[(size_t)i], trace_base_, t.ev[i]) == hipSuccess;
-        if (ok) ts.push_back(a); else (void)hipGetLastError();
+        for (int i = 0; i < (t.head ? 8 : 6) && ok; ++i) ok = hipEventElapsedTime(&ln.a[(size_t)i], trace_base_, t.ev[i]) == hipSuccess;
+        if (ok) ts.push_back(ln); else (void)hipGetLastError();
     }
     for (size_t i = 0; i < ts.size(); ++i) {
-        const auto &a = ts[i];
-        const bool fe_in_prev = i > 0 && a[0] * 1e3f < ts[i - 1][3] * 1e3f && a[1] * 1e3f > ts[i - 1][2] * 1e3f;
-        const bool sr_in_next = i + 1 < ts.size() && a[5] > ts[i + 1][2] && a[4] < ts[i + 1][3];
-        fprintf(f, "%4zu %5d %2d  %10.1f %10.1f  %10.1f %10.1f  %10.1f %10.1f   %s %s\n", i, trace_[i].m, trace_[i].T, a[0] * 1e3, a[1] * 1e3, a[2] * 1e3, a[3] * 1e3, a[4] * 1e3, a[5] * 1e3,
-                fe_in_prev ? "FE<prevLY" : "-", sr_in_next ? "SR<nextLY" : "-");
+        const auto &a = ts[i].a;
+        const bool fe_in_prev = i > 0 && a[0] * 1e3f < ts[i - 1].a[3] * 1e3f && a[1] * 1e3f > ts[i - 1].a[2] * 1e3f;
+        const bool sr_in_next = i + 1 < ts.size() && a[5] > ts[i + 1].a[2] && a[4] < ts[i + 1].a[3];
+        const bool hd_in_prev = ts[i].head && i > 0 && a[6] < ts[i - 1].a[3];
+        fprintf(f, "%4zu %5d %2d  %10.1f %10.1f  %10.1f %10.1f  %10.1f %10.1f   %s %s   %10.1f %10.1f  %s %s\n", i, ts[i].m, ts[i].T, a[0] * 1e3, a[1] * 1e3, a[2] * 1e3, a[3] * 1e3, a[4] * 1e3, a[5] * 1e3,
+                fe_in_prev ? "FE<prevLY" : "-", sr_in_next ? "SR<nextLY" : "-", a[6] * 1e3, a[7] * 1e3, ts[i].offered ? "offered" : "-", hd_in_prev ? "HD<prevLYend" : "-");
     }
     fclose(f);
 }
@@ -1111,8 +1124,7 @@
         gclk_used_ = 0;
     }
     SwPlan &p = sw_plans_[key];
-    build_sw_chain(p, p.one, m, T, false);
-    if (ramp_mode_ != 0 && !gclk_) build_sw_chain(p, p.split, m, T, true);
+    build_sw_chain(p, m, T);
     return p;
 }
 
@@ -1132,49 +1144,40 @@
 
 void Engine::ramp_counts(uint64_t *hosted, uint64_t *eligible)
 {
-    unsigned h = 0;
-    {
-        HipLegacyLock legacy;
-        if (hipSetDevice(cfg_.device) == hipSuccess) HIP_CHECK(hipMemcpy(&h, &ramp_d_->hosted, sizeof h, hipMemcpyDeviceToHost));
-    }
-    *hosted = h; *eligible = ramp_eligible_.load(std::memory_order_relaxed);
-}
-
-void Engine::build_sw_chain(SwPlan &p, SwPlan::Chain &c, int m, int T, bool ramp)
-{
+    *hosted = ramp_hosted_.load(std::memory_order_relaxed); *eligible = ramp_eligible_.load(std::memory_order_relaxed);
+}
+
+void Engine::build_sw_chain(SwPlan &p, int m, int T)
+{
+    SwPlan::Chain &c = p.one;
     const NetDims &d = L_.dims;
     const int L = d.n_layers;
-    const int par = flight_parity_;
     const int tk = f16_tile_ ? 2 : tile_ok();
     auto needs_rows = [&](int kind, int n) {
         const int kz = kind == 1 ? kz_hr() : kz_ff2();
         return (kind == 1 || kind == 3) && tk && (tk == 2 || gemm_tile_planned(m, d.d_model, kz, n)) && !gemm_fullk(m, d.d_model, kz, false, n, tk);
     };
-    std::vector<RampStep> window;
-    if (ramp && m <= RAMP_MAX_M && T <= RAMP_MAX_T) {
-        window = ramp_window(L, T, RAMP_R);
-        for (const RampStep &s : window) if (needs_rows(1, s.own + (int)s.guests.size()) || needs_rows(3, s.own + (int)s.guests.size())) { window.clear(); break; }
-    }
-    if (ramp) p.hosts = !window.empty();
+    const std::vector<RampStep> window = ramp_mode_ != 0 && !gclk_ ? ramp_window(L, T, RAMP_R, 1 << 30) : std::vector<RampStep>();
+    bool separate = !window.empty();
+    for (const RampStep &s : window) if (needs_rows(1, s.own + (int)s.guests.size()) || needs_rows(3, s.own + (int)s.guests.size())) separate = false;
+    const int window_macro = separate ? window[0].macro : 0;
     std::vector<GemmArgs> items;
     std::vector<RowArgs> rows;
     for (int W = 0; W <= T + L; ++W) {
-        const RampStep *host = nullptr; int wj = 0;
-        for (size_t j = 0; j < window.size(); ++j) if (window[j].macro == W) { host = &window[j]; wj = (int)j; }
-        if (host && wj == 0) { SwPlan::Batch b; b.off = c.host.size(); b.n = 0; b.macro = W; b.kind = 4; b.roff = c.rhost.size(); b.rn = 0; c.batches.push_back(b); }
+        if (separate && W == RAMP_R + 1) p.head_end = c.batches.size();
+        if (separate && W == window_macro) p.window_at = c.batches.size();
         for (int kind = 0; kind < 4; ++kind) {
             items.clear(); rows.clear();
             int n_act = 0;
             for (int l = 0; l < L; ++l) { const int t = W - 1 - l; if (t >= 0 && t < T) ++n_act; }
             if (n_act == 0) continue;
-            if (host) n_act += (int)host->guests.size();
             const int kz = kind == 1 ? kz_hr() : kz_ff2();
             const bool split = needs_rows(kind, n_act);
-            auto problem = [&](int l, int t, const int *run_flag) {
+            if (split && separate && (W <= RAMP_R || W >= window_macro)) separate = false;
+            auto problem = [&](int l, int t) {
                 const size_t r0 = (size_t)t * m;
                 GemmArgs g = kind == 0 ? args_gates(l, r0, m, GATES_ALL) : kind == 1 ? args_whr(l, r0, m) : kind == 2 ? args_ff1(l, r0, m) : args_ff2(l, r0, m);
                 if (kind == 0 && cfg_.precision == 0) g.tile_ok = gates_tile_rows((long)m * n_act) ? 2 : 0;
-                if (run_flag) { g.run_flag = run_flag; g.run_gen = 1; }
                 if (split) {
                     float *ws = ws_ + r0 * d.d_model;
                     rows.push_back(row_form(g, ws, ws_mstride_, gemm_partials(m, d.d_model, kz, n_act, tk)));
@@ -1185,12 +1188,7 @@
             for (int l = 0; l < L; ++l) {
                 const int t = W - 1 - l;
                 if (t < 0 || t >= T) continue;
-                problem(l, t, ramp && W <= RAMP_R ? &ramp_d_->head_live[par] : nullptr);
-            }
-            if (host) {
-                select_parity(1 - par);
-                for (const auto &lt : host->guests) problem(lt.first, lt.second, &ramp_d_->guest_live[par][wj][lt.second]);
-                select_parity(par);
+                problem(l, t);
             }
             std::vector<int> groups;
             {
@@ -1202,11 +1200,11 @@
             size_t first = 0;
             for (size_t gi = 0; gi < groups.size(); ++gi) {
                 const int gn = groups[gi];
-                if (kind == 0 && !ramp && gclk_ && gclk_slots_ && gclk_used_ < GCLK_SLOTS) {
+                if (kind == 0 && gclk_ && gclk_slots_ && gclk_used_ < GCLK_SLOTS) {
                     p.stamp_slots.push_back(std::make_pair(gclk_used_, (long)m * gn)); p.stamp_n.push_back(gn);
                     for (int i = 0; i < gn; ++i) items[first + (size_t)i].stamp = gclk_slots_ + (size_t)gclk_used_ * STAMP_WORDS;
                     ++gclk_used_;
-                } else if (kind == 0 && !ramp && gclk_ && gclk_slots_ && !gclk_warned_) {
+                } else if (kind == 0 && gclk_ && gclk_slots_ && !gclk_warned_) {
                     gclk_warned_ = true; LOGW("engine: the gates clock is out of stamp slots (%d): the gates launches of further plans are not timed", GCLK_SLOTS);
                 }
                 SwPlan::Batch b; b.off = c.host.size(); b.n = gn; b.macro = W; b.kind = kind; b.roff = c.rhost.size(); b.rn = gi == 0 ? (int)rows.size() : 0;
@@ -1218,6 +1216,7 @@
             }
         }
     }
+    if (!separate) p.head_end = p.window_at = 0;
     m_touched();
     c.dev = dmalloc<GemmArgs>(c.host.size());
     HIP_CHECK(hipMemcpyAsync(c.dev, c.host.data(), c.host.size() * sizeof(GemmArgs), hipMemcpyHostToDevice, stream_));
@@ -1230,7 +1229,7 @@
 void Engine::free_sw_plans()
 {
     if (!sw_plans_.empty()) LOGI("engine: feed wavefront plans emptied (%zu plans)", sw_plans_.size());
-    for (auto &p : sw_plans_) for (SwPlan::Chain *c : {&p.second.one, &p.second.split}) { if (c->dev) (void)hipFree(c->dev); if (c->rdev) (void)hipFree(c->rdev); }
+    for (auto &p : sw_plans_) for (SwPlan::Chain *c : {&p.second.one}) { if (c->dev) (void)hipFree(c->dev); if (c->rdev) (void)hipFree(c->rdev); }
     sw_graphs_.clear(); sw_plans_.clear();
 }
 
@@ -1242,12 +1241,18 @@
         launch_advance(advance_args(m, T), st);
         encoder_front(0, m * T, step_d_ + 3 * MB, nullptr, st, part == 0 ? ws_fe_ : ws_);
     }
-    if (part < 0 || part == 1) {
+    if (part < 0 || part == 1 || part >= 3) {
         static const int cls_of[4] = {T_GATES, T_GEMM_OTHER, T_GEMM_OTHER, T_GEMM_OTHER};
-        const SwPlan::Chain &c = p.layers(part == 1);
-        for (size_t bi = 0; bi < c.batches.size(); ++bi) {
+        const SwPlan::Chain &c = p.one;
+        const size_t b0 = part == 6 ? p.window_at : part >= 4 ? p.head_end : 0, b1 = part == 3 ? p.head_end : part == 5 ? p.window_at : c.batches.size();
+        for (size_t bi = b0; bi < b1; ++bi) {
             const SwPlan::Batch &b = c.batches[bi];
-            if (b.kind == 4) { launch_ramp_latch(ramp_d_, flight_parity_, m, st); continue; }
+            if (part == 4 && bi == p.window_at) {
+                hipStreamCaptureStatus cap = hipStreamCaptureStatusNone;
+                HIP_CHECK(hipStreamIsCapturing(st, &cap));
+                if (cap == hipStreamCaptureStatusActive) HIP_CHECK(hipEventRecordWithFlags(window_ev_[flight_parity_], st, hipEventRecordExternal));
+                else HIP_CHECK(hipEventRecord(window_ev_[flight_parity_], st));
+            }
             timed_begin(cls_of[b.kind]); launch_gemm_z(c.host.data() + b.off, b.n, c.dev + b.off, st); timed_end(cls_of[b.kind]);
             if (b.rn > 0) { timed_begin(T_ROW); launch_row_z(c.rhost.data() + b.roff, b.rn, c.rdev + b.roff, st); timed_end(T_ROW); }
         }
@@ -1295,8 +1300,11 @@
     if (graphs && !sw_graphs_.find(sw_key(m, T, split ? 1 : 0)))
         capture_both_parities([&]() {
             const SwPlan &pl = sw_plan(m, T);
-            if (split) for (int part = 0; part < 3; ++part) cached_graph(sw_graphs_, sw_key(m, T, 1 + part), on[part], [&]() { run_sw_chain(m, T, false, pl, part, on[part]); });
-            else cached_graph(sw_graphs_, sw_key(m, T), stream_, [&]() { run_sw_chain(m, T, false, pl, -1, stream_); });
+            if (split) {
+                const bool sep = pl.head_end > 0 && on[0] == f_stream_;
+                for (int part = 0; part < 3; ++part) if (part != 1 || !sep) cached_graph(sw_graphs_, sw_key(m, T, 1 + part), on[part], [&]() { run_sw_chain(m, T, false, pl, part, on[part]); });
+                if (sep) for (int part : {3, 4, 5, 6}) if (part == 3 || (part == 4) == event_node_) cached_graph(sw_graphs_, sw_key(m, T, 1 + part), on[part > 3], [&]() { run_sw_chain(m, T, false, pl, part, on[part > 3]); });
+            } else cached_graph(sw_graphs_, sw_key(m, T), stream_, [&]() { run_sw_chain(m, T, false, pl, -1, stream_); });
         });
     if (split) { launch_split_feed(m, T, on[0]); return; }
     general_prologue();
@@ -1311,21 +1319,32 @@
     } else if (f_unseen_by_m_) { join(stream_, f_stream_); f_unseen_by_m_ = false; }
     if (m_unseen_by_s_) { join(s_stream_, stream_); m_unseen_by_s_ = false; }
     StreamTrace *tr = trace_slot();
-    auto part = [&](int i, hipStream_t st) {
+    auto part = [&](int i, int key_part, hipStream_t st) {
         if (tr) HIP_CHECK(hipEventRecord(tr->ev[2 * i], st));
-        HIP_CHECK(hipGraphLaunch(sw_graphs_.find(sw_key(m, T, 1 + i)), st));
+        HIP_CHECK(hipGraphLaunch(sw_graphs_.find(sw_key(m, T, key_part)), st));
         if (tr) HIP_CHECK(hipEventRecord(tr->ev[2 * i + 1], st));
     };
-    part(0, fe);
-    if (ramp_mode_ != 0) {
-        const bool hostable = ramp_mode_ == 1 && fe == f_stream_ && m_quiet_.load(std::memory_order_acquire);
-        if (hostable) ramp_eligible_.fetch_add(1, std::memory_order_relaxed);
-        launch_ramp_ready(ramp_d_, flight_parity_, m, T, hostable ? 1 : 0, fe);
+    const bool sep = fe == f_stream_ && sw_graphs_.find(sw_key(m, T, 4)) != nullptr;
+    part(0, 1, fe);
+    if (sep) {
+        const bool offered = ramp_mode_ == 1 && last_window_ && m_quiet_.load(std::memory_order_acquire);
+        if (offered) {
+            ramp_eligible_.fetch_add(1, std::memory_order_relaxed); ramp_hosted_.fetch_add(1, std::memory_order_relaxed);
+            HIP_CHECK(hipStreamWaitEvent(f_stream_, last_window_, 0));
+        } else join(f_stream_, stream_);
+        part(3, 4, fe);
+        if (tr) { tr->head = true; tr->offered = offered; }
     }
     if (fe == f_stream_) { join(stream_, f_stream_); f_unseen_by_m_ = false; }
-    part(1, stream_);
-    if (ramp_mode_ != 0) m_quiet_.store(true, std::memory_order_release);
-    join(s_stream_, stream_); part(2, s_stream_);
+    if (sep && !event_node_) {
+        if (tr) HIP_CHECK(hipEventRecord(tr->ev[2], stream_));
+        HIP_CHECK(hipGraphLaunch(sw_graphs_.find(sw_key(m, T, 6)), stream_));
+        HIP_CHECK(hipEventRecord(window_ev_[flight_parity_], stream_));
+        HIP_CHECK(hipGraphLaunch(sw_graphs_.find(sw_key(m, T, 7)), stream_));
+        if (tr) HIP_CHECK(hipEventRecord(tr->ev[3], stream_));
+    } else part(1, sep ? 5 : 2, stream_);
+    if (ramp_mode_ != 0) { last_window_ = sep ? window_ev_[flight_parity_] : nullptr; m_quiet_.store(true, std::memory_order_release); }
+    join(s_stream_, stream_); part(2, 3, s_stream_);
     if (tr) { tr->m = m; tr->T = T; tr->used = true; }
     s_unseen_by_m_ = true; flight_tail_s_ = true;
     if (fe != f_stream_) m_unseen_by_f_ = true;
diff --git a/april_asr_amd/csrc/engine.h b/april_asr_amd/csrc/engine.h
--- a/april_asr_amd/csrc/engine.h
+++ b/april_asr_amd/csrc/engine.h
@@ -62,6 +62,10 @@
     std::map<Key, hipGraphExec_t> map_; std::map<std::pair<int, int>, int> uses_;
 };
 
+#ifndef APRIL_RAMP_R
+#define APRIL_RAMP_R 2
+#endif
+constexpr int RAMP_R = APRIL_RAMP_R;
 struct RampStep { int macro = 0, own = 0; std::vector<std::pair<int, int>> guests; };
 std::vector<RampStep> ramp_window(int L, int T, int R, int max_problems = 3);
 
@@ -221,22 +225,20 @@
         struct Batch { size_t off; int n, macro, kind; size_t roff; int rn; };
         struct Chain { std::vector<GemmArgs> host; GemmArgs *dev = nullptr; std::vector<Batch> batches; std::vector<RowArgs> rhost; RowArgs *rdev = nullptr; };
         Chain one;
-        Chain split;
-        bool hosts = false;
-        const Chain &layers(bool split_feed) const { return split_feed && !split.batches.empty() ? split : one; }
+        size_t head_end = 0, window_at = 0;
         std::vector<std::pair<int, long>> stamp_slots; std::vector<int> stamp_n;
     };
-    GraphCache::Key graph_key(int m, int T = 0, int part = 0) const { return {m, T, flight_parity_ * 4 + part}; }
+    GraphCache::Key graph_key(int m, int T = 0, int part = 0) const { return {m, T, flight_parity_ * 8 + part}; }
     GraphCache::Key sw_key(int m, int T, int part = 0) const { return graph_key(gclk_ ? -m : m, T, part); }
     SwPlan &sw_plan(int m, int T);
-    void build_sw_chain(SwPlan &p, SwPlan::Chain &c, int m, int T, bool ramp);
+    void build_sw_chain(SwPlan &p, int m, int T);
     void free_sw_plans();
     void run_sw_chain(int m, int T, bool dump_logits, const SwPlan &p, int part, hipStream_t st);
     int stage_step(int m, int T, const int *slots, const int *ring_tails, const int *now_ms); void read_back_logits(int k, int rows, float *out);
     template <typename Chain> hipGraphExec_t cached_graph(GraphCache &cache, const GraphCache::Key &key, hipStream_t st, Chain &&chain);
     template <typename Capture> void capture_both_parities(Capture &&capture);
     void run_feed_wavefront(int m, int T, bool dump_logits); void run_layer_major(int m, int T, bool dump_logits); void launch_split_feed(int m, int T, hipStream_t fe);
-    struct StreamTrace { hipEvent_t ev[6] = {nullptr, nullptr, nullptr, nullptr, nullptr, nullptr}; int m = 0, T = 0; bool used = false; };
+    struct StreamTrace { hipEvent_t ev[8] = {nullptr, nullptr, nullptr, nullptr, nullptr, nullptr, nullptr, nullptr}; int m = 0, T = 0; bool used = false, head = false, offered = false; };
     std::deque<StreamTrace> trace_; hipEvent_t trace_base_ = nullptr;
     StreamTrace *trace_slot();
     void dump_stream_trace();
@@ -318,10 +320,12 @@
     bool overlap_hint_ = false;
     int split_streams_ = 2;
     int ramp_mode_ = 1;
-    RampState *ramp_d_ = nullptr;
+    hipEvent_t window_ev_[2] = {nullptr, nullptr};
+    bool event_node_ = false;
+    hipEvent_t last_window_ = nullptr;
     std::atomic<bool> m_quiet_{false};
     void m_touched() { m_quiet_.store(false, std::memory_order_release); }
-    std::atomic<uint64_t> ramp_eligible_{0};
+    std::atomic<uint64_t> ramp_eligible_{0}, ramp_hosted_{0};
     float *xb_buf_[2] = {nullptr, nullptr}, *u_buf_[2] = {nullptr, nullptr}, *ff_buf_[2] = {nullptr, nullptr};
     uint16_t *xb16_buf_[2] = {nullptr, nullptr}, *u16_buf_[2] = {nullptr, nullptr}, *ff16_buf_[2] = {nullptr, nullptr};
     float *y_buf_[2] = {nullptr, nullptr}, *ssq_buf_[2] = {nullptr, nullptr}, *eout_lm_buf_[2] = {nullptr, nullptr}, *ws_fe_ = nullptr, *ws_sr_ = nullptr;
diff --git a/april_asr_amd/csrc/kernels.h b/april_asr_amd/csrc/kernels.h
--- a/april_asr_amd/csrc/kernels.h
+++ b/april_asr_amd/csrc/kernels.h
@@ -114,18 +114,6 @@
 };
 void launch_row(const RowArgs &r, hipStream_t s);
 void launch_row_z(const RowArgs *host_args, int n, const RowArgs *dev_args, hipStream_t s);
-
-constexpr int RAMP_R = 2;
-struct RampState {
-    unsigned long long ready[2];
-    int head_live[2];
-    int guest_live[2][RAMP_R][RAMP_R];
-    unsigned generation;
-    unsigned hosted;
-};
-constexpr int RAMP_MAX_M = 0xFFFFF, RAMP_MAX_T = 0xFF;
-void launch_ramp_ready(RampState *rs, int q, int m, int T, int hostable, hipStream_t s);
-void launch_ramp_latch(RampState *rs, int p, int m, hipStream_t s);
 
 struct StepRecord { int32_t idx; float max_val; float blank_val; uint32_t flags; };
 constexpr int kConfMaxAlt = 8;
diff --git a/april_asr_amd/csrc/kernels_misc.hip b/april_asr_amd/csrc/kernels_misc.hip
--- a/april_asr_amd/csrc/kernels_misc.hip
+++ b/april_asr_amd/csrc/kernels_misc.hip
@@ -86,44 +86,6 @@
     case ROW_RESID_SSQ: hipLaunchKernelGGL(row_zkernel<ROW_RESID_SSQ>, grid, block, 0, s, dev_args); break;
     default: hipLaunchKernelGGL(row_zkernel<ROW_SLOT_STORE>, grid, block, 0, s, dev_args); break;
     }
-}
-
-__global__ __launch_bounds__(64) void ramp_ready_kernel(RampState *rs, int q, int m, int T, int hostable)
-{
-    if (threadIdx.x != 0) return;
-    __hip_atomic_store(&rs->head_live[q], 1, __ATOMIC_RELAXED, __HIP_MEMORY_SCOPE_AGENT);
-    const unsigned g = __hip_atomic_load(&rs->generation, __ATOMIC_RELAXED, __HIP_MEMORY_SCOPE_AGENT) + 1u;
-    __hip_atomic_store(&rs->generation, g, __ATOMIC_RELAXED, __HIP_MEMORY_SCOPE_AGENT);
-    __builtin_amdgcn_fence(__ATOMIC_RELEASE, "agent");
-    asm volatile("s_waitcnt vmcnt(0)" ::: "memory");
-    const unsigned long long rec = ((unsigned long long)g << 32) | ((unsigned long long)(unsigned)m << 12) | ((unsigned long long)(unsigned)T << 4) | (unsigned long long)(hostable & 1);
-    __hip_atomic_store(&rs->ready[q], rec, __ATOMIC_RELAXED, __HIP_MEMORY_SCOPE_AGENT);
-}
-
-__global__ __launch_bounds__(64) void ramp_latch_kernel(RampState *rs, int p, int m)
-{
-    if (threadIdx.x != 0) return;
-    const unsigned long long mine = __hip_atomic_load(&rs->ready[p], __ATOMIC_RELAXED, __HIP_MEMORY_SCOPE_AGENT);
-    const unsigned long long next = __hip_atomic_load(&rs->ready[1 - p], __ATOMIC_RELAXED, __HIP_MEMORY_SCOPE_AGENT);
-    const unsigned g = (unsigned)(mine >> 32);
-    const int next_m = (int)((next >> 12) & RAMP_MAX_M), next_T = (int)((next >> 4) & RAMP_MAX_T);
-    const bool host = (unsigned)(next >> 32) == g + 1u && next_m == m && (int)((mine >> 12) & RAMP_MAX_M) == m && (next & 1ull) != 0;
-    if (host) {
-        __builtin_amdgcn_fence(__ATOMIC_ACQUIRE, "agent");
-        __hip_atomic_store(&rs->head_live[1 - p], 0, __ATOMIC_RELAXED, __HIP_MEMORY_SCOPE_AGENT);
-        rs->hosted += 1u;
-    }
-    for (int j = 1; j <= RAMP_R; ++j)
-        for (int t = 0; t < RAMP_R; ++t) rs->guest_live[p][j - 1][t] = (host && t < j && t < next_T) ? 1 : 0;
-}
-
-void launch_ramp_ready(RampState *rs, int q, int m, int T, int hostable, hipStream_t s)
-{
-    hipLaunchKernelGGL(ramp_ready_kernel, dim3(1), dim3(64), 0, s, rs, q, m, T, hostable);
-}
-void launch_ramp_latch(RampState *rs, int p, int m, hipStream_t s)
-{
-    hipLaunchKernelGGL(ramp_latch_kernel, dim3(1), dim3(64), 0, s, rs, p, m);
 }
 
 __device__ __forceinline__ void dec_embed_row(const DecEmbedParams &p, int tok0, int tok1, float *out)
```

Measured after the change: 20040. No clear change (-0.0%).
